# walaj/SeqLib

Measured on AMD Instinct MI355X. Metric: aligned reads/sec (150 bp) via BWAAligner, higher is better.
Workload: dtype int32

## Files before the change

### seqlib_amd/csrc/dev_ext_lane.h

```cpp
#pragma once
#include "dev_seed4.h"
#include "dev_ext_reg.h"
#include "dev_lane_rows.h"

struct alignas(8) LaneJob {
    int64_t s_rbeg, rmax0, rmax1;
    uint64_t q_off;
    int l_query, s_qbeg, s_len, rid;
    float frac_rep;
    int out;
    int r, c;
};

#define LANE_SCORE_LIMIT 16000


struct LaneBases {
    const DevRef &R;
    const uint8_t *query;
    RWin rw;
    __device__ __forceinline__ int q(int j) const { return (int)query[j]; }
    __device__ __forceinline__ int t(int64_t p) { return text_at(R, p, rw); }
};

__device__ __forceinline__ void lane_exits_add(unsigned int *dst, unsigned int mine, int lane)
{
    const unsigned int sum = (unsigned int)__builtin_amdgcn_readlane(dpp_incl_add_scan((int)mine), WAVE - 1);
    if (dst && sum && lane == 0) atomicAdd(dst, sum);
}

template <typename L>
__device__ DReg lane_extend_core(const DevRef &R, const slx_opt &opt, const MatRows &mr, const uint8_t *query, int l_query, int s_qbeg, int s_len,
                                 int64_t s_rbeg, int64_t rmax0, int64_t rmax1, int rid, float frac_rep, L &eh, int row_exit, unsigned int &n_exit)
{
    DReg a;
    a.rb = a.re = 0; a.qb = a.qe = 0; a.sub = a.csub = a.sub_n = 0; a.seedcov = 0; a.secondary = 0;
    a.n_comp = 0; a.hash = 0;
    int aw0 = opt.w, aw1 = opt.w;
    a.w = opt.w; a.rid = rid;
    a.score = a.truesc = s_len * opt.a; a.qb = 0; a.rb = s_rbeg;
    const int qe = s_qbeg + s_len;
    const int64_t re0 = s_rbeg + s_len;
    a.qe = l_query; a.re = re0;
    LaneSide sd[2];
    sd[0].qlen = s_qbeg; sd[0].tlen = (int)(s_rbeg - rmax0); sd[0].q0 = s_qbeg - 1; sd[0].t0 = s_rbeg - 1; sd[0].end_bonus = opt.pen_clip5;
    sd[1].qlen = l_query - qe; sd[1].tlen = (int)(rmax1 - re0); sd[1].q0 = qe; sd[1].t0 = re0; sd[1].end_bonus = opt.pen_clip3;
    LaneBases bases{R, query, {0, -1}};
    lane_rows_extend(sd, s_len * opt.a, opt, mr, eh, bases, [&](int side, const LaneRes &er) {
        if (side == 0) {
            aw0 = er.aw;
            a.score = er.score;
            if (er.gscore <= 0 || er.gscore <= a.score - opt.pen_clip5) { a.qb = s_qbeg - er.qle; a.rb = s_rbeg - er.tle; a.truesc = a.score; }
            else { a.qb = 0; a.rb = s_rbeg - er.gtle; a.truesc = er.gscore; }
        } else {
            aw1 = er.aw;
            const int sc0 = a.score;
            a.score = er.score;
            if (er.gscore <= 0 || er.gscore <= a.score - opt.pen_clip3) { a.qe = qe + er.qle; a.re = re0 + er.tle; a.truesc += a.score - sc0; }
            else { a.qe = l_query; a.re = re0 + er.gtle; a.truesc += er.gscore - sc0; }
        }
    }, row_exit ? EXT_ROW_EXIT_RELAXED : EXT_ROW_EXIT_OFF, &n_exit);
    a.w = aw0 > aw1 ? aw0 : aw1;
    a.seedlen0 = s_len;
    a.frac_rep = frac_rep;
    return a;
}

template <int MAXQ>
__global__ void __launch_bounds__(64) k_cand_lane_prep(DevRef R, Chunk ck, DevOpt dopt, const int *heavy, const unsigned int *n_heavy, const unsigned int *job_off, LaneJob *jobs)
{
    const slx_opt &opt = dopt.o;
    const int lane = threadIdx.x;
    __shared__ int gap_lut[MAXQ + 2];
    for (int q = lane; q < MAXQ + 2; q += WAVE) gap_lut[q] = dev_cal_max_gap(opt, q);
    __syncthreads();
    auto max_gap_of = [&](int q) { return gap_lut[q < 0 ? 0 : (q > MAXQ + 1 ? MAXQ + 1 : q)]; };
    const int64_t l_pac = R.l_pac;
    const unsigned int nh = (unsigned int)__builtin_amdgcn_readfirstlane((int)*n_heavy);
    for (unsigned int s = blockIdx.x; s < nh; s += gridDim.x) {
        const int r = heavy[s];
        const int base = __builtin_amdgcn_readfirstlane(ck.cand_base[r]);
        if (base < 0 || job_off[s + 1] == job_off[s]) continue;
        const unsigned int job0 = job_off[s];
        const ReadWS w = make_ws_uniform(ck, r);
        const uint64_t q_off = ck.offs[r];
        const int l_query = (int)(ck.offs[r + 1] - q_off);
        const int n_chn = ck.n_chain[r];
        const float frac_rep = ck.frac_rep[r];
        unsigned int running = 0;
        for (int cb = 0; cb < n_chn; cb += WAVE) {
            const int ci = cb + lane;
            const int c = ci < n_chn ? w.ia[ci] : -1;
            const int n = c >= 0 ? w.c_n[c] : 0;
            int incl = n;
            for (int d = 1; d < WAVE; d <<= 1) { const int u = __shfl_up(incl, d, WAVE); if (lane >= d) incl += u; }
            const unsigned int my = running + (unsigned int)(incl - n);
            running += (unsigned int)__shfl(incl, WAVE - 1, WAVE);
            if (n <= 0) continue;
            const int *cs = w.c_w + w.c_first[c];
            int64_t rmax0 = l_pac << 1, rmax1 = 0;
            for (int i = 0; i < n; ++i) {
                const int sd = cs[i];
                const int qb = w.s_qbeg(sd), sl = w.s_len(sd);
                const int64_t b = w.s_rbeg[sd] - (qb + max_gap_of(qb));
                const int64_t e = w.s_rbeg[sd] + sl + ((l_query - qb - sl) + max_gap_of(l_query - qb - sl));
                rmax0 = rmax0 < b ? rmax0 : b;
                rmax1 = rmax1 > e ? rmax1 : e;
            }
            rmax0 = rmax0 > 0 ? rmax0 : 0;
            rmax1 = rmax1 < l_pac << 1 ? rmax1 : l_pac << 1;
            const int64_t first_rbeg = w.s_rbeg[cs[0]];
            if (rmax0 < l_pac && l_pac < rmax1) {
                if (first_rbeg < l_pac) rmax1 = l_pac; else rmax0 = l_pac;
            }
            {
                int is_rev;
                const int rid = dev_pos2rid(R, dev_depos(R, first_rbeg, &is_rev));
                int64_t far_beg = R.ann_off[rid], far_end = far_beg + R.ann_len[rid];
                if (is_rev) { const int64_t t = far_beg; far_beg = (l_pac << 1) - far_end; far_end = (l_pac << 1) - t; }
                rmax0 = rmax0 > far_beg ? rmax0 : far_beg;
                rmax1 = rmax1 < far_end ? rmax1 : far_end;
            }
            const int rid_c = w.c_rid[c];
            for (int i = 0; i < n; ++i) {
                const int sd = cs[i];
                LaneJob j;
                j.s_rbeg = w.s_rbeg[sd]; j.rmax0 = rmax0; j.rmax1 = rmax1; j.q_off = q_off; j.l_query = l_query;
                j.s_qbeg = w.s_qbeg(sd); j.s_len = w.s_len(sd); j.rid = rid_c; j.frac_rep = frac_rep; j.out = base + sd; j.r = r; j.c = c;
                jobs[job0 + my + (unsigned int)i] = j;
            }
        }
    }
}

template <typename L>
__global__ void __launch_bounds__(64) k_ext_lanes(DevRef R, Chunk ck, DevOpt dopt, const unsigned int *n_heavy, const unsigned int *job_off, unsigned int *queue,
                                                   const LaneJob *jobs, DReg *cand, int cols)
{
    const slx_opt &opt = dopt.o;
    const int lane = threadIdx.x;
    const MatRows mr = make_matrows(opt.mat);
    extern __shared__ uint32_t lane_lds[];
    L row;
    row.init(lane_lds, cols, lane);
    const unsigned int nh = (unsigned int)__builtin_amdgcn_readfirstlane((int)*n_heavy);
    const unsigned int n_jobs = nh ? (unsigned int)__builtin_amdgcn_readfirstlane((int)job_off[nh]) : 0u;
    unsigned int exit_cnt = 0;
    for (;;) {
        const unsigned int base = wave_take(queue, (unsigned int)WAVE);
        if (base >= n_jobs) break;
        const unsigned int job = base + (unsigned int)lane;
        if (job < n_jobs) {
            const LaneJob j = jobs[job];
            const uint8_t *query = ck.codes + j.q_off;
            DReg a = lane_extend_core<L>(R, opt, mr, query, j.l_query, j.s_qbeg, j.s_len, j.s_rbeg, j.rmax0, j.rmax1, j.rid, j.frac_rep, row, ck.ext_row_exit, exit_cnt);
            const ReadWS w = make_ws(ck, j.r);
            const int n = w.c_n[j.c];
            const int *cs = w.c_w + w.c_first[j.c];
            int cov = 0;
            for (int i = 0; i < n; ++i) {
                const int t = cs[i];
                const int t_qbeg = w.s_qbeg(t), t_len = w.s_len(t);
                const int64_t t_rbeg = w.s_rbeg[t];
                if (t_qbeg >= a.qb && t_qbeg + t_len <= a.qe && t_rbeg >= a.rb && t_rbeg + t_len <= a.re) cov += t_len;
            }
            a.seedcov = cov;
            cand[j.out] = a;
        }
    }
    lane_exits_add(ck.ext_exits, exit_cnt, lane);
}

__device__ __forceinline__ int first_job_bin(const FirstJob &j, int max_len)
{
    const int left = j.s_qbeg, right = j.l_query - j.s_qbeg - j.s_len;
    const float w = sqrtf((float)(left * left + right * right));
    int b = (int)(w * 64.f / (float)(max_len > 0 ? max_len : 1));
    b = b > 63 ? 63 : (b < 0 ? 0 : b);
    return 63 - b;
}
__global__ void __launch_bounds__(256) k_first_bin_count(const FirstJob *jobs, const unsigned int *dp_list, const unsigned int *n_dp, int max_len, unsigned int *bins)
{
    __shared__ unsigned int s[64];
    if (threadIdx.x < 64) s[threadIdx.x] = 0;
    __syncthreads();
    const unsigned int n = *n_dp;
    for (unsigned int t = blockIdx.x * blockDim.x + threadIdx.x; t < n; t += gridDim.x * blockDim.x) atomicAdd(&s[first_job_bin(jobs[dp_list[t]], max_len)], 1u);
    __syncthreads();
    if (threadIdx.x < 64 && s[threadIdx.x]) atomicAdd(&bins[threadIdx.x], s[threadIdx.x]);
}
__global__ void k_first_bin_scan(unsigned int *bins)
{
    if (blockIdx.x == 0 && threadIdx.x == 0) { unsigned int acc = 0; for (int b = 0; b < 64; ++b) { bins[64 + b] = acc; acc += bins[b]; } }
}
__global__ void __launch_bounds__(256) k_first_bin_scatter(const FirstJob *jobs, const unsigned int *dp_list, const unsigned int *n_dp, int max_len, unsigned int *bins, unsigned int *out)
{
    __shared__ unsigned int s_cnt[64], s_base[64];
    const unsigned int n = *n_dp;
    for (unsigned int t0 = blockIdx.x * blockDim.x; t0 < n; t0 += gridDim.x * blockDim.x) {
        if (threadIdx.x < 64) s_cnt[threadIdx.x] = 0;
        __syncthreads();
        const unsigned int t = t0 + threadIdx.x;
        int b = -1;
        unsigned int job = 0, my = 0;
        if (t < n) { job = dp_list[t]; b = first_job_bin(jobs[job], max_len); my = atomicAdd(&s_cnt[b], 1u); }
        __syncthreads();
        if (threadIdx.x < 64 && s_cnt[threadIdx.x]) s_base[threadIdx.x] = atomicAdd(&bins[64 + threadIdx.x], s_cnt[threadIdx.x]);
        __syncthreads();
        if (b >= 0) out[s_base[b] + my] = job;
        __syncthreads();
    }
}

template <typename L>
__global__ void __launch_bounds__(64) k_first_lanes(DevRef R, Chunk ck, DevOpt dopt, unsigned int *queue, const FirstJob *jobs, DReg *first, const unsigned int *list,
                                                     const unsigned int *n_list, int cols, unsigned int *n_ran)
{
    const slx_opt &opt = dopt.o;
    const int lane = threadIdx.x;
    const MatRows mr = make_matrows(opt.mat);
    extern __shared__ uint32_t lane_lds[];
    L row;
    row.init(lane_lds, cols, lane);
    const unsigned int n_jobs = (unsigned int)__builtin_amdgcn_readfirstlane((int)*n_list);
    unsigned int exit_cnt = 0;
    for (;;) {
        const unsigned int base = wave_take(queue, (unsigned int)WAVE);
        if (base >= n_jobs) break;
        const unsigned int t = base + (unsigned int)lane;
        if (t < n_jobs) {
            const unsigned int job = list[t];
            const FirstJob j = jobs[job];
            const DReg a = lane_extend_core<L>(R, opt, mr, ck.codes + j.q_off, j.l_query, j.s_qbeg, j.s_len, j.s_rbeg, j.rmax0, j.rmax1, j.rid, j.frac_rep, row, ck.ext_row_exit, exit_cnt);
            first[job] = a;
        }
        if (lane == 0) atomicAdd(n_ran, n_jobs - base < (unsigned int)WAVE ? n_jobs - base : (unsigned int)WAVE);
    }
    lane_exits_add(ck.ext_exits, exit_cnt, lane);
}

template <typename QF, typename TF>
__device__ __forceinline__ bool lane_diag_extend(int qlen, QF qf, int tlen, TF tf, const slx_opt &o, const MatRows &mr, int amax, int h0, ExtResult &out)
{
    if (tlen < qlen || qlen > 3 * WAVE || qlen < 1) return false;
    if ((long long)h0 + (long long)qlen * amax >= (1 << 22)) return false;
    const int oe_del = o.o_del + o.e_del, oe_ins = o.o_ins + o.e_ins;
    const int oe = oe_del < oe_ins ? oe_del : oe_ins;
    int loss = 0, run = h0, best = h0, best_p = -1;
    for (int p = 0; p < qlen; ++p) {
        const int t = tf(p), q = qf(p);
        const uint32_t rowp = t == 0 ? mr.packed[0] : t == 1 ? mr.packed[1] : t == 2 ? mr.packed[2] : mr.packed[3];
        const int row4 = t == 0 ? mr.q4[0] : t == 1 ? mr.q4[1] : t == 2 ? mr.q4[2] : mr.q4[3];
        const int sc = q < 4 ? __builtin_amdgcn_sbfe((int)rowp, (uint32_t)q << 3, 8u) : row4;
        loss += amax - sc;
        if (loss > oe - 1) return false;
        run += sc;
        if (run > best) { best = run; best_p = p; }
    }
    if (h0 <= loss) return false;
    out.score = best; out.qle = best_p + 1; out.tle = best_p + 1; out.gtle = qlen; out.gscore = run; out.max_off = 0;
    return true;
}

__global__ void __launch_bounds__(256) k_first_diag(DevRef R, Chunk ck, DevOpt dopt, int n, const unsigned int *first_off, unsigned int cap, const FirstJob *jobs, DReg *first,
                                                    unsigned int *dp_list, unsigned int *n_dp)
{
    const slx_opt &opt = dopt.o;
    const MatRows mr = make_matrows(opt.mat);
    int amax = 0;
    for (int i = 0; i < 25; ++i) amax = amax > opt.mat[i] ? amax : opt.mat[i];
    unsigned int n_jobs = first_off[n];
    if (n_jobs > cap) n_jobs = cap;
    const unsigned int job = blockIdx.x * blockDim.x + threadIdx.x;
    if (job >= n_jobs) return;
    const FirstJob j = jobs[job];
    if (j.l_query <= 0) return;
    const uint8_t *codes = ck.codes;
    QWin qw; qw.bits = 0; qw.chunk = 0xffffffffu;
    RWin rw; rw.bits = 0; rw.chunk = -1;
    DReg a;
    a.rb = a.re = 0; a.qb = a.qe = 0; a.sub = a.csub = a.sub_n = 0; a.seedcov = 0; a.secondary = 0;
    a.n_comp = 0; a.hash = 0;
    a.score = a.truesc = -1; a.rid = j.rid;
    const int aw_ext = ((opt.w >> 1) + (opt.w >> 2)) > 0 ? opt.w : opt.w << 1;
    int aw0 = opt.w, aw1 = opt.w;
    bool ok = true;
    const int s_qbeg = j.s_qbeg, s_len = j.s_len, l_query = j.l_query;
    const int64_t s_rbeg = j.s_rbeg;
    if (s_qbeg) {
        aw0 = aw_ext;
        ExtResult er;
        ok = lane_diag_extend(s_qbeg, [&](int p) { return q_at(codes, j.q_off + (uint64_t)(s_qbeg - 1 - p), qw); }, (int)(s_rbeg - j.rmax0),
                              [&](int t) { return text_at(R, s_rbeg - 1 - t, rw); }, opt, mr, amax, s_len * opt.a, er);
        if (ok) {
            a.score = er.score;
            if (er.gscore <= 0 || er.gscore <= a.score - opt.pen_clip5) { a.qb = s_qbeg - er.qle; a.rb = s_rbeg - er.tle; a.truesc = a.score; }
            else { a.qb = 0; a.rb = s_rbeg - er.gtle; a.truesc = er.gscore; }
        }
    } else { a.score = a.truesc = s_len * opt.a; a.qb = 0; a.rb = s_rbeg; }
    if (ok) {
        if (s_qbeg + s_len != l_query) {
            aw1 = aw_ext;
            const int sc0 = a.score, qe = s_qbeg + s_len;
            const int64_t re0 = s_rbeg + s_len;
            ExtResult er;
            ok = lane_diag_extend(l_query - qe, [&](int p) { return q_at(codes, j.q_off + (uint64_t)(qe + p), qw); }, (int)(j.rmax1 - re0),
                                  [&](int t) { return text_at(R, re0 + t, rw); }, opt, mr, amax, sc0, er);
            if (ok) {
                a.score = er.score;
                if (er.gscore <= 0 || er.gscore <= a.score - opt.pen_clip3) { a.qe = qe + er.qle; a.re = re0 + er.tle; a.truesc += a.score - sc0; }
                else { a.qe = l_query; a.re = re0 + er.gtle; a.truesc += er.gscore - sc0; }
            }
        } else { a.qe = l_query; a.re = s_rbeg + s_len; }
    }
    if (ok) {
        a.w = aw0 > aw1 ? aw0 : aw1;
        a.seedlen0 = s_len;
        a.frac_rep = j.frac_rep;
        first[job] = a;
    } else dp_list[wave_fetch_inc(n_dp)] = job;
}
```

### seqlib_amd/csrc/dev_lane_rows.h

```cpp
#pragma once
#include <stdint.h>
#include <stddef.h>
#if defined(__HIPCC__)
#define LROW_FN __host__ __device__ __forceinline__
#define LROW_M __host__ __device__ __forceinline__
#else
#define LROW_FN static inline
#define LROW_M inline
#endif
#ifndef WAVE
#define WAVE 64
#endif

template <typename O>
LROW_FN int ext_tail_bound0(const O &o, int qlen, int h0, int amax)
{
    if (o.o_del < 0 || o.e_del < 0 || o.o_ins < 0 || o.e_ins < 0) return 0x7fffffff;
    const long long b = (long long)h0 + (long long)qlen * (amax > 0 ? amax : 0) - o.o_del - o.e_del;
    return b > 0x3fffffff ? 0x7fffffff : (int)b;
}
LROW_FN bool ext_tail_done(int b, int max, int gscore) { return b <= max && (b > 0 ? b : 0) < gscore; }

#define EXT_ROW_EXIT_OFF 0
#define EXT_ROW_EXIT_STRICT 1
#define EXT_ROW_EXIT_RELAXED 2
template <typename O>
LROW_FN bool ext_row_exit_ok(const O &o, int qlen, int w, int h0)
{
    if (o.o_del < 0 || o.e_del < 0 || o.o_ins < 0 || o.e_ins < 0) return false;
    return w + 1 >= qlen || (long long)h0 - o.o_ins - o.e_ins - (long long)(w + 1) * o.e_ins <= 0;
}
LROW_FN int ext_row_bound(int m, int hb, int apos, int qlen, int beg, int tlen, int i)
{
    const int a = qlen - beg, b = tlen - 1 - i;
    const int k = a < b ? a : b;
    return (m > hb ? m : hb) + apos * (k > 0 ? k : 0);
}
LROW_FN bool ext_row_done(int U, int max, int gscore, int end_bonus) { return (end_bonus >= 0 && U <= max - end_bonus) || ext_tail_done(U, max, gscore); }

struct LaneWide {
    uint32_t *eh;
    static LROW_M size_t bytes(int cols) { return (size_t)cols * WAVE * 4; }
    LROW_M void init(uint32_t *base, int, int lane) { eh = base + lane; }
    LROW_M void put_all(int j, int h, int e, int q) { eh[j * WAVE] = (uint32_t)h | (uint32_t)e << 14 | (uint32_t)q << 28; }
    LROW_M uint32_t get(int j) const { return eh[j * WAVE]; }
    LROW_M int q_of(uint32_t v, int) const { return (int)(v >> 28); }
    static LROW_M int h_of(uint32_t v) { return (int)(v & 0x3fffu); }
    static LROW_M int e_of(uint32_t v) { return (int)((v >> 14) & 0x3fffu); }
    LROW_M void put(int j, int h, int e, uint32_t old) { eh[j * WAVE] = (uint32_t)h | (uint32_t)e << 14 | (old & 0xf0000000u); }
    static LROW_M bool zero(uint32_t v) { return (v & 0x0fffffffu) == 0; }
};
struct LaneNarrow {
    uint16_t *eh;
    uint32_t *qa;
    static LROW_M size_t bytes(int cols) { return (size_t)cols * WAVE * 2 + (size_t)((cols + 7) / 8) * WAVE * 4; }
    LROW_M void init(uint32_t *base, int cols, int lane) { eh = (uint16_t *)base + lane; qa = base + (size_t)cols * WAVE / 2 + lane; }
    LROW_M void put_all(int j, int h, int e, int q)
    {
        eh[j * WAVE] = (uint16_t)(h | e << 8);
        uint32_t w = (j & 7) ? qa[(j >> 3) * WAVE] : 0u;
        w |= (uint32_t)q << ((j & 7) * 4);
        qa[(j >> 3) * WAVE] = w;
    }
    LROW_M uint32_t get(int j) const { return eh[j * WAVE]; }
    LROW_M int q_of(uint32_t, int j) const { return (int)((qa[(j >> 3) * WAVE] >> ((j & 7) * 4)) & 7u); }
    static LROW_M int h_of(uint32_t v) { return (int)(v & 0xffu); }
    static LROW_M int e_of(uint32_t v) { return (int)(v >> 8); }
    LROW_M void put(int j, int h, int e, uint32_t) { eh[j * WAVE] = (uint16_t)(h | e << 8); }
    static LROW_M bool zero(uint32_t v) { return v == 0; }
};

struct LaneSide { int qlen, tlen, q0, end_bonus; int64_t t0; };
struct LaneRes { int score, qle, tle, gtle, gscore, max_off, aw; };

template <typename L, typename F, typename O, typename MR, typename D>
LROW_FN void lane_rows_extend(const LaneSide s[2], int h0, const O &o, const MR &mr, L &row, F &fetch, D done, int row_exit = EXT_ROW_EXIT_STRICT,
                              unsigned int *n_exit = nullptr)
{
    const int o_del = o.o_del, e_del = o.e_del, o_ins = o.o_ins, e_ins = o.e_ins, zdrop = o.zdrop;
    const int oe_del = o_del + e_del, oe_ins = o_ins + e_ins;
    int amax = 0;
    for (int i = 0; i < 25; ++i) amax = amax > o.mat[i] ? amax : o.mat[i];
    int side = s[0].qlen > 0 ? 0 : (s[1].qlen > 0 ? 1 : 2), trial = 0, prev = -1;
    bool fresh = true;
    int qlen = 0, tlen = 0, q0 = 0, dir = 0, w = 0, aw = 0, tail_top = 0, exit_bonus = -1;
    bool exit_ok = false;
    const int apos = amax > 0 ? amax : 0;
    int64_t t0 = 0;
    int max = 0, max_i = -1, max_j = -1, max_ie = -1, gscore = -1, max_off = 0, beg = 0, end = 0, i = 0;
    while (side < 2) {
        if (fresh) {
            fresh = false;
            const int end_bonus = side ? s[1].end_bonus : s[0].end_bonus;
            qlen = side ? s[1].qlen : s[0].qlen; tlen = side ? s[1].tlen : s[0].tlen; q0 = side ? s[1].q0 : s[0].q0; t0 = side ? s[1].t0 : s[0].t0;
            dir = side ? 1 : -1;
            aw = o.w << trial;
            for (int j = 0; j <= qlen; ++j) {
                const int v = h0 - oe_ins - (j - 1) * e_ins;
                const int h = j == 0 ? h0 : (v > 0 ? v : 0);
                row.put_all(j, h, 0, j < qlen ? fetch.q(q0 + dir * j) : 0);
            }
            w = aw;
            int max_ins = (int)((double)(qlen * amax + end_bonus - o_ins) / e_ins + 1.);
            max_ins = max_ins > 1 ? max_ins : 1;
            w = w < max_ins ? w : max_ins;
            int max_del = (int)((double)(qlen * amax + end_bonus - o_del) / e_del + 1.);
            max_del = max_del > 1 ? max_del : 1;
            w = w < max_del ? w : max_del;
            tail_top = ext_tail_bound0(o, qlen, h0, amax);
            exit_ok = row_exit != EXT_ROW_EXIT_OFF && ext_row_exit_ok(o, qlen, w, h0);
            exit_bonus = row_exit == EXT_ROW_EXIT_RELAXED ? end_bonus : -1;
            max = h0;
            max_i = -1; max_j = -1; max_ie = -1; gscore = -1; max_off = 0; beg = 0; end = qlen; i = 0;
        }
        bool stop = i >= tlen || (i >= qlen && ext_tail_done(tail_top - (i - qlen) * e_del, max, gscore));
        if (!stop) {
            const int t = fetch.t(t0 + (int64_t)(dir * i));
            const uint32_t rowp = t == 0 ? mr.packed[0] : t == 1 ? mr.packed[1] : t == 2 ? mr.packed[2] : t == 3 ? mr.packed[3] : mr.packed[4];
            const int row4 = t == 0 ? mr.q4[0] : t == 1 ? mr.q4[1] : t == 2 ? mr.q4[2] : t == 3 ? mr.q4[3] : mr.q4[4];
            int f = 0, m = 0, mj = -1;
            if (beg < i - w) beg = i - w;
            if (end > i + w + 1) end = i + w + 1;
            if (end > qlen) end = qlen;
            int h1 = 0;
            if (beg == 0) { h1 = h0 - (o_del + e_del * (i + 1)); if (h1 < 0) h1 = 0; }
            const int hb = h1;
            uint32_t cur = beg < end ? row.get(beg) : 0u;
            for (int j = beg; j < end; ++j) {
                const uint32_t nxt = row.get(j + 1);
                int M = L::h_of(cur), e = L::e_of(cur);
                const uint32_t q = (uint32_t)row.q_of(cur, j);
#if defined(__HIP_DEVICE_COMPILE__)
                const int sc = q < 4 ? __builtin_amdgcn_sbfe((int)rowp, q << 3, 8u) : row4;
#else
                const int sc = q < 4 ? (int)(int8_t)(rowp >> (q << 3)) : row4;
#endif
                M = M ? M + sc : 0;
                int h = M > e ? M : e;
                h = h > f ? h : f;
                const int hl = h1;
                h1 = h;
                mj = m > h ? mj : j;
                m = m > h ? m : h;
                int t2 = M - oe_del; t2 = t2 > 0 ? t2 : 0;
                e -= e_del; e = e > t2 ? e : t2;
                row.put(j, hl, e, cur);
                t2 = M - oe_ins; t2 = t2 > 0 ? t2 : 0;
                f -= e_ins; f = f > t2 ? f : t2;
                cur = nxt;
            }
            row.put(end, h1, 0, beg < end ? cur : row.get(end));
            if ((end > beg ? end : beg) == qlen) {
                max_ie = gscore > h1 ? max_ie : i;
                gscore = gscore > h1 ? gscore : h1;
            }
            if (m == 0) stop = true;
            else if (m > max) {
                max = m; max_i = i; max_j = mj;
                const int off = mj - i < 0 ? i - mj : mj - i;
                max_off = max_off > off ? max_off : off;
            } else if (zdrop > 0) {
                if (i - max_i > mj - max_j) { if (max - m - ((i - max_i) - (mj - max_j)) * e_del > zdrop) stop = true; }
                else { if (max - m - ((mj - max_j) - (i - max_i)) * e_ins > zdrop) stop = true; }
            }
            if (!stop) {
                int j;
                for (j = beg; j < end && L::zero(row.get(j)); ++j) {}
                beg = j;
                for (j = end; j >= beg && L::zero(row.get(j)); --j) {}
                end = j + 2 < qlen ? j + 2 : qlen;
                if (exit_ok && ext_row_done(ext_row_bound(m, beg == 0 ? hb : 0, apos, qlen, beg, tlen, i), max, gscore, exit_bonus)) {
                    stop = true;
                    if (n_exit) ++*n_exit;
                }
                ++i;
            }
        }
        if (stop) {
            fresh = true;
            const int before = trial ? prev : (side ? h0 : -1);
            if (trial == 0 && !(max == before || max_off < (aw >> 1) + (aw >> 2))) { prev = max; trial = 1; }
            else {
                LaneRes r;
                r.score = max; r.qle = max_j + 1; r.tle = max_i + 1; r.gtle = max_ie + 1; r.gscore = gscore; r.max_off = max_off; r.aw = aw;
                done(side, r);
                if (side == 0) h0 = max;
                side = side == 0 && s[1].qlen > 0 ? 1 : 2;
                trial = 0;
            }
        }
    }
}
```

### seqlib_amd/csrc/slx_align.hip

```cpp
#include <hip/hip_runtime.h>
#include <hipcub/hipcub.hpp>
#include <chrono>
#include <cmath>
#include <functional>
#include <unistd.h>
#include <cstdio>
#include <cstdlib>
#include <cstring>
#include <algorithm>
#include <mutex>
#include <string>
#include <thread>
#include <type_traits>
#include <vector>
#include "slx_internal.h"
#include "dev_seed4.h"
#include "dev_fin.h"
#include "dev_ext_wave.h"
#include "dev_ext_reg.h"
#include "dev_ext_lane.h"
#include "dev_ext_block.h"
#include "dev_ext_seg.h"
#include "dev_fin2.h"
#include "dev_chain_coop.h"
// ... 187 lines not shown
    if (al->rep_k <= 0 || al->rep_k > 31 || !al->have_dense || al->host_idx->seq_len < 1024) return SLX_OK;
    uint64_t bits = 1ull << 20;
    while (bits < al->host_idx->seq_len * 8ull) bits <<= 1;
    while (al->d_rep.ensure(bits / 8) != SLX_OK) {
        (void)hipGetLastError();
        bits >>= 1;
        if (bits < al->host_idx->seq_len || bits < (1ull << 20)) { al->d_rep.release(); return SLX_OK; }
    }
    HIPCHK(hipMemsetAsync(al->d_rep.p, 0, bits / 8, al->stream));
    DevFM<I> fm = fm_of<I>(al);
    fm.sa_dense = al->d_sa_dense.as<I>();
    hipLaunchKernelGGL(k_rep_filter<I>, dim3(al->n_cu * 64), dim3(256), 0, al->stream, fm, al->ref, al->rep_k, al->d_rep.as<uint32_t>(), bits - 1);
    HIPCHK(hipGetLastError());
    HIPCHK(slx_wait_stream(al->stream));
    al->rep_mask = bits - 1;
    return SLX_OK;
}

#define SLX_MAX_WORKERS 8
static int env_hw_queues() { const char *e = getenv("GPU_MAX_HW_QUEUES"); const int v = e ? atoi(e) : 0; return v > 0 ? v : 4; }

static int default_workers()
{
    if (const char *e = getenv("SEQLIB_AMD_WORKERS")) { const int v = atoi(e); if (v >= 1 && v <= SLX_MAX_WORKERS) return v; }
    return 3;
}

static int make_worker_stream(slx_aligner *al, Worker *wk)
{
    if (al->stream_prio) {
        int least = 0, greatest = 0;
        HIPCHK(hipDeviceGetStreamPriorityRange(&least, &greatest));
        HIPCHK(hipStreamCreateWithPriority(&wk->stream, hipStreamNonBlocking, greatest));
    } else HIPCHK(hipStreamCreateWithFlags(&wk->stream, hipStreamNonBlocking));
    return SLX_OK;
}

static int set_seed_stream(slx_aligner *al, Worker *wk)
{
    if (wk->seed_stream) { HIPCHK(slx_wait_stream(wk->seed_stream)); HIPCHK(hipStreamDestroy(wk->seed_stream)); wk->seed_stream = nullptr; }
    if (al->seed_free_cus <= 0) return SLX_OK;
    const int words = (al->n_cu + 31) / 32;
    std::vector<uint32_t> mask((size_t)words, 0u);
    for (int cu = 0; cu < al->n_cu; ++cu)
        if ((cu & 31) < 32 - al->seed_free_cus) mask[(size_t)(cu >> 5)] |= 1u << (cu & 31);
    HIPCHK(hipExtStreamCreateWithCUMask(&wk->seed_stream, (uint32_t)words, mask.data()));
    if (!wk->ev_seed_in) HIPCHK(hipEventCreateWithFlags(&wk->ev_seed_in, hipEventDisableTiming));
    if (!wk->ev_seed_out) HIPCHK(hipEventCreateWithFlags(&wk->ev_seed_out, hipEventDisableTiming));
    return SLX_OK;
}

static int add_worker(slx_aligner *al)
{
    Worker *wk = new Worker();
    wk->id = (int)al->workers.size();
    wk->collect();
    al->workers.push_back(wk);
    { const int rc = make_worker_stream(al, wk); if (rc != SLX_OK) return rc; }
    { const int rc = set_seed_stream(al, wk); if (rc != SLX_OK) return rc; }
    HIPCHK(hipHostMalloc((void **)&wk->h_mail, 256, hipHostMallocDefault));
    for (int b = 0; b < 6; ++b) HIPCHK(hipEventCreate(&wk->dbg_ev[b]));
    for (int i = 0; i <= SLX_N_STAGES; ++i) HIPCHK(hipEventCreate(&wk->ev[i]));
    for (int i = 0; i < 6; ++i) HIPCHK(hipEventCreate(&wk->ev_probe[i]));
    return SLX_OK;
}

static int aligner_init(slx_aligner *al, const slx_index *idx, const int *devices, int n_dev)
{
    al->device = (devices && n_dev > 0) ? devices[0] : 0;
    if (!(devices && n_dev > 0)) (void)hipGetDevice(&al->device);
    HIPCHK(hipSetDevice(al->device));
    hipDeviceProp_t prop;
    HIPCHK(hipGetDeviceProperties(&prop, al->device));
    al->n_cu = prop.multiProcessorCount;
    al->max_threads = al->n_cu * al->threads_per_cu;
    int rcw;
    al->n_workers = default_workers();
    al->hw_queues = env_hw_queues();
    for (int k = 0; k < al->n_workers; ++k) if ((rcw = add_worker(al)) != SLX_OK) return rcw;
    HIPCHK(hipStreamCreateWithFlags(&al->stream, hipStreamNonBlocking));
    al->host_idx = idx;
    int rc;
    if ((rc = al->d_bwt.ensure(idx->bwt.size() * 4 + 64)) != SLX_OK) return rc;
    HIPCHK(hipMemcpy(al->d_bwt.p, idx->bwt.data(), idx->bwt.size() * 4, hipMemcpyHostToDevice));
    if ((rc = al->d_sa_samp.ensure(idx->sa.size() * 8)) != SLX_OK) return rc;
    HIPCHK(hipMemcpy(al->d_sa_samp.p, idx->sa.data(), idx->sa.size() * 8, hipMemcpyHostToDevice));
    al->wide = idx->seq_len + 1 >= (1ULL << 32);
    if ((rc = al->wide ? upload_fm<uint64_t>(al) : upload_fm<uint32_t>(al)) != SLX_OK) return rc;
    if ((rc = al->d_pac.ensure(idx->pac.size() + 16)) != SLX_OK) return rc;
    HIPCHK(hipMemcpy(al->d_pac.p, idx->pac.data(), idx->pac.size(), hipMemcpyHostToDevice));
    std::vector<int64_t> aoff; std::vector<int32_t> alen;
    for (const slx_ann &a : idx->anns) { aoff.push_back(a.offset); alen.push_back(a.len); }
    if ((rc = al->d_ann_off.ensure(aoff.size() * 8 + 8)) != SLX_OK) return rc;
    if ((rc = al->d_ann_len.ensure(alen.size() * 4 + 8)) != SLX_OK) return rc;
    HIPCHK(hipMemcpy(al->d_ann_off.p, aoff.data(), aoff.size() * 8, hipMemcpyHostToDevice));
    HIPCHK(hipMemcpy(al->d_ann_len.p, alen.data(), alen.size() * 4, hipMemcpyHostToDevice));
    al->ref.pac = al->d_pac.as<uint8_t>();
    al->ref.l_pac = idx->l_pac;
    al->ref.n_seqs = (int)idx->anns.size();
    al->ref.ann_off = al->d_ann_off.as<int64_t>();
    al->ref.ann_len = al->d_ann_len.as<int32_t>();
    {
        std::vector<uint8_t> alt;
        bool any = false;
        for (const slx_ann &a : idx->anns) { alt.push_back(a.is_alt ? 1 : 0); any = any || a.is_alt; }
        al->ref.ann_alt = nullptr;
        if (any) {
            if ((rc = al->d_ann_alt.ensure(alt.size() + 8)) != SLX_OK) return rc;
            HIPCHK(hipMemcpy(al->d_ann_alt.p, alt.data(), alt.size(), hipMemcpyHostToDevice));
            al->ref.ann_alt = al->d_ann_alt.as<uint8_t>();
        }
    }
    if ((rc = al->wide ? find_text_is_pac<uint64_t>(al) : find_text_is_pac<uint32_t>(al)) != SLX_OK) return rc;
    if ((rc = al->wide ? build_rep_filter<uint64_t>(al) : build_rep_filter<uint32_t>(al)) != SLX_OK) return rc;
    const int LUT_N = SLX_LOG_LUT_N;
    std::vector<double> lut((size_t)LUT_N);
    lut[0] = -INFINITY;
    for (int i = 1; i < LUT_N; ++i) lut[(size_t)i] = log((double)i);
    if ((rc = al->d_loglut.ensure((size_t)LUT_N * 8)) != SLX_OK) return rc;
    HIPCHK(hipMemcpy(al->d_loglut.p, lut.data(), (size_t)LUT_N * 8, hipMemcpyHostToDevice));
    return SLX_OK;
}


static std::mutex g_live_mu;
static int g_live_aligners = 0;
static void pin_pool_release_all();

static int create_one(const slx_index *idx, int device, bool current, slx_aligner **out)
{
    slx_aligner *al = new slx_aligner();
    { std::lock_guard<std::mutex> g(g_live_mu); ++g_live_aligners; }
    const int rc = aligner_init(al, idx, current ? nullptr : &device, current ? 0 : 1);
    if (rc != SLX_OK) { slx_aligner_free(al); return rc; }
    *out = al;
    return SLX_OK;
}

extern "C" int slx_device_count(void)
{
    int ndev = 0;
    if (hipGetDeviceCount(&ndev) != hipSuccess) { (void)hipGetLastError(); return 0; }
    return ndev;
}

extern "C" int slx_aligner_create(const slx_index *idx, const int *devices, int n_dev, slx_aligner **out)
{
    if (!out) return SLX_EINVAL;
    *out = nullptr;
    if (!idx) { slx_set_error("slx_aligner_create: index is null"); return SLX_EINVAL; }
    const int ndev = slx_device_count();
    if (ndev == 0) {
        slx_set_error("no HIP device: the BWAAligner hot path runs on MI355X only (no CPU fallback)");
        return SLX_ENODEVICE;
    }
    if (n_dev < 0 || (n_dev > 0 && !devices)) { slx_set_error("slx_aligner_create: bad device list"); return SLX_EINVAL; }
    for (int i = 0; i < n_dev; ++i)
        if (devices[i] < 0 || devices[i] >= ndev) { slx_set_error("slx_aligner_create: device %d is not one of the %d visible", devices[i], ndev); return SLX_EINVAL; }
    if (n_dev <= 1) return create_one(idx, n_dev ? devices[0] : 0, n_dev == 0, out);
    slx_aligner *grp = new slx_aligner();
    grp->is_group = true;
    grp->subs.assign((size_t)n_dev, nullptr);
    grp->host_idx = idx;
    std::vector<int> rcs((size_t)n_dev, SLX_OK);
    std::vector<std::string> errs((size_t)n_dev);
    std::vector<std::thread> th;
    for (int i = 0; i < n_dev; ++i)
        th.emplace_back([&, i]() {
            rcs[(size_t)i] = create_one(idx, devices[i], false, &grp->subs[(size_t)i]);
            if (rcs[(size_t)i] != SLX_OK) errs[(size_t)i] = slx_last_error();
        });
    for (auto &t : th) t.join();
    for (int i = 0; i < n_dev; ++i)
        if (rcs[(size_t)i] != SLX_OK) {
            slx_set_error("device %d: %s", devices[i], errs[(size_t)i].c_str());
            const int rc = rcs[(size_t)i];
            slx_aligner_free(grp);
            return rc;
        }
    *out = grp;
    return SLX_OK;
}

extern "C" void slx_aligner_free(slx_aligner *al)
{
    if (!al) return;
    if (al->is_group) {
        for (slx_aligner *sub : al->subs) slx_aligner_free(sub);
        delete al;
        return;
    }
    (void)hipSetDevice(al->device);
    DevBuf *bufs[] = {&al->d_bwt, &al->d_occ, &al->d_sup, &al->d_lut, &al->d_rep, &al->d_sa_samp, &al->d_sa_dense, &al->d_pac, &al->d_ann_off, &al->d_ann_len, &al->d_ann_alt, &al->d_loglut, &al->o_hit_off,
                      &al->o_rid, &al->o_pos, &al->o_flag, &al->o_mapq, &al->o_score, &al->o_nm, &al->o_na, &al->o_ncig, &al->o_cig_off, &al->o_cigar, &al->o_xa, &al->o_sub,
                      &al->st_bases, &al->st_offs, &al->st_pack};
    for (DevBuf *b : bufs) b->release();
    for (Worker *wk : al->workers) {
        for (DevBuf *b : wk->all) b->release();
        for (int i = 0; i <= SLX_N_STAGES; ++i) if (wk->ev[i]) (void)hipEventDestroy(wk->ev[i]);
        for (int i = 0; i < 6; ++i) if (wk->dbg_ev[i]) (void)hipEventDestroy(wk->dbg_ev[i]);
        for (int i = 0; i < 6; ++i) if (wk->ev_probe[i]) (void)hipEventDestroy(wk->ev_probe[i]);
        if (wk->h_mail) (void)hipHostFree(wk->h_mail);
        if (wk->stream) (void)hipStreamDestroy(wk->stream);
        if (wk->seed_stream) (void)hipStreamDestroy(wk->seed_stream);
        if (wk->ev_seed_in) (void)hipEventDestroy(wk->ev_seed_in);
        if (wk->ev_seed_out) (void)hipEventDestroy(wk->ev_seed_out);
        delete wk;
    }
    if (al->h_bounce) (void)hipHostFree(al->h_bounce);
    if (al->stream) (void)hipStreamDestroy(al->stream);
    delete al;
    bool last;
    { std::lock_guard<std::mutex> g(g_live_mu); last = --g_live_aligners == 0; }
    if (last) pin_pool_release_all();
}

extern "C" int slx_aligner_set(slx_aligner *al, const char *key, int64_t value)
{
    if (!al || !key) return SLX_EINVAL;
    if (al->is_group) {
        std::lock_guard<std::mutex> call(al->call_mu);
        for (slx_aligner *sub : al->subs) { const int rc = slx_aligner_set(sub, key, value); if (rc != SLX_OK) return rc; }
        return SLX_OK;
    }
    std::lock_guard<std::mutex> call(al->call_mu);
    if (!strcmp(key, "chunk_reads")) { if (value < 1) return SLX_EINVAL; al->chunk_reads = value; }
    else if (!strcmp(key, "cap_intv")) { if (value < 1) return SLX_EINVAL; al->cap_intv = (int)value; }
    else if (!strcmp(key, "dense_sa")) al->dense_sa = value != 0;
    else if (!strcmp(key, "wide_index")) {
        const bool want = value != 0 || al->host_idx->seq_len + 1 >= (1ULL << 32);
        if (want != al->wide) {
            HIPCHK(hipSetDevice(al->device));
            al->wide = want;
            int rc = want ? upload_fm<uint64_t>(al) : upload_fm<uint32_t>(al);
            if (rc != SLX_OK) return rc;
            if ((rc = want ? build_rep_filter<uint64_t>(al) : build_rep_filter<uint32_t>(al)) != SLX_OK) return rc;
        }
    }
    else if (!strcmp(key, "chain_mode")) al->chain_mode = (int)value;
    else if (!strcmp(key, "keep_stages")) al->keep_stages = (int)value;
    else if (!strcmp(key, "lut_k")) {
        if (value != 0 && value != -1 && (value < 2 || value > 14)) return SLX_EINVAL;
        al->lut_k = (int)value;
        (void)hipSetDevice(al->device);
        return al->wide ? build_lut<uint64_t>(al) : build_lut<uint32_t>(al);
    }
    else if (!strcmp(key, "cand_mode")) al->cand_mode = (int)value;
    else if (!strcmp(key, "cand_seeds")) { if (value < 1) return SLX_EINVAL; al->cand_seeds = (int)value; }
    else if (!strcmp(key, "heavy_sorted")) al->heavy_sorted = (int)value;
    else if (!strcmp(key, "ext_split")) al->ext_split = (int)value;
    else if (!strcmp(key, "coop_lim1")) { if (value < 1) return SLX_EINVAL; al->coop_lim1 = (int)value; }
    else if (!strcmp(key, "coop_lim2")) { if (value < 1) return SLX_EINVAL; al->coop_lim2 = (int)value; }
    else if (!strcmp(key, "long_coop")) al->long_coop = value != 0;
    else if (!strcmp(key, "long_seed3")) al->long_seed3 = value != 0;
    else if (!strcmp(key, "long_predict")) al->long_predict = value != 0;
    else if (!strcmp(key, "long_block")) { if (value < 0 || value > (1 << 24)) return SLX_EINVAL; al->long_block = (int)value; }
    else if (!strcmp(key, "long_guess")) al->long_guess = value != 0;
    else if (!strcmp(key, "long_seg")) al->long_seg = value != 0;
    else if (!strcmp(key, "bwd_direct")) al->bwd_direct = value != 0;
    else if (!strcmp(key, "xseg_wave_min")) { if (value < 0) return SLX_EINVAL; al->xseg_wave_min = (int)value; }
    else if (!strcmp(key, "xseg_fail")) { if (value < 0) return SLX_EINVAL; al->xseg_fail = (int)value; }
    else if (!strcmp(key, "long_budget")) { if (value < 0 || value > (1 << 20)) return SLX_EINVAL; al->long_budget = (int)value; }
    else if (!strcmp(key, "regs_big")) { if (value < 2) return SLX_EINVAL; al->regs_big = (int)value; }
    else if (!strcmp(key, "regs_defer")) al->regs_defer = value != 0;
    else if (!strcmp(key, "hits_wave")) al->hits_wave = value != 0;
    else if (!strcmp(key, "cig_fast_coop")) al->cig_fast_coop = value != 0;
    else if (!strcmp(key, "cig_lane_il")) al->cig_lane_il = value != 0;
    else if (!strcmp(key, "small_coop")) al->small_coop = value != 0;
    else if (!strcmp(key, "small_spread")) al->small_spread = value != 0;
    else if (!strcmp(key, "chain_sorted")) al->chain_sorted = value != 0;
    else if (!strcmp(key, "regs_sorted")) al->regs_sorted = value != 0;
    else if (!strcmp(key, "cand_top")) { if (value < 0) return SLX_EINVAL; al->cand_top = (int)value; }
    else if (!strcmp(key, "cand_rep_max")) { if (value < 0) return SLX_EINVAL; al->cand_rep_max = (int)value; }
    else if (!strcmp(key, "cand_rep")) { if (value < -1 || value > 101) return SLX_EINVAL; al->cand_rep = (int)value; }
    else if (!strcmp(key, "cand_lanes")) { if (value < -1 || value > 1) return SLX_EINVAL; al->cand_lanes = (int)value; }
    else if (!strcmp(key, "cig_lanes")) al->cig_lanes = value != 0;
    else if (!strcmp(key, "first_diag")) al->first_diag = value != 0;
    else if (!strcmp(key, "first_lanes")) al->first_lanes = value != 0;
    else if (!strcmp(key, "chain_lds")) al->chain_lds = value != 0;
    else if (!strcmp(key, "lane_narrow")) al->lane_narrow = value != 0;
    else if (!strcmp(key, "lane_pad")) al->lane_pad = (int)value;
    else if (!strcmp(key, "cand_lane_seeds")) { if (value < 1) return SLX_EINVAL; al->cand_lane_seeds = (int)value; }
    else if (!strcmp(key, "cand_cap")) { if (value < 1) return SLX_EINVAL; al->cand_cap = (int)value; }
    else if (!strcmp(key, "split_min")) al->split_min = (int)value;
    else if (!strcmp(key, "heavy_seeds")) { if (value < 1) return SLX_EINVAL; al->heavy_seeds = (int)value; }
    else if (!strcmp(key, "workers")) {
        if (value < 1 || value > SLX_MAX_WORKERS) return SLX_EINVAL;
        HIPCHK(hipSetDevice(al->device));
        while ((int)al->workers.size() < (int)value) { const int rc = add_worker(al); if (rc != SLX_OK) return rc; }
        al->n_workers = (int)value;
    }
    else if (!strcmp(key, "min_split")) { if (value < 1) return SLX_EINVAL; al->min_split = value; }
    else if (!strcmp(key, "seed_quota")) { if (value < 0 || value > (1 << 24)) return SLX_EINVAL; al->seed_quota = (int)value; }
    else if (!strcmp(key, "rep_k")) {
        if (value < 0 || value > 31) return SLX_EINVAL;
        al->rep_k = (int)value;
        HIPCHK(hipSetDevice(al->device));
        return al->wide ? build_rep_filter<uint64_t>(al) : build_rep_filter<uint32_t>(al);
    }
    else if (!strcmp(key, "top_heavy")) al->top_heavy = value != 0;
    else if (!strcmp(key, "top_reuse")) al->top_reuse = value != 0;
    else if (!strcmp(key, "walk_stage")) al->walk_stage = value != 0;
    else if (!strcmp(key, "ext_row_exit")) al->ext_row_exit = value != 0;
    else if (!strcmp(key, "p2_items")) al->p2_items = value != 0;
    else if (!strcmp(key, "p2_coop")) al->p2_coop = value != 0;
    else if (!strcmp(key, "p2_items_cap")) al->p2_items_cap = (int)value;
    else if (!strcmp(key, "seed_free_cus")) {
        if (value < 0 || value > 24) return SLX_EINVAL;
        HIPCHK(hipSetDevice(al->device));
        al->seed_free_cus = (int)value;
        for (Worker *wk : al->workers) { const int rc = set_seed_stream(al, wk); if (rc != SLX_OK) return rc; }
    }
    else if (!strcmp(key, "stream_prio")) {
        if (value < 0 || value > 1) return SLX_EINVAL;
        HIPCHK(hipSetDevice(al->device));
        al->stream_prio = (int)value;
        for (Worker *wk : al->workers) {
            HIPCHK(slx_wait_stream(wk->stream));
            HIPCHK(hipStreamDestroy(wk->stream));
            wk->stream = nullptr;
            const int rc = make_worker_stream(al, wk);
            if (rc != SLX_OK) return rc;
        }
    }
    else if (!strcmp(key, "threads")) { if (value < 64) return SLX_EINVAL; al->max_threads = (int)value; }
    else if (!strcmp(key, "zarena_bytes")) { if (value < 1024) return SLX_EINVAL; al->zcap = (unsigned long long)value; }
    else if (!strcmp(key, "z_start") || !strcmp(key, "cig_start")) {
        if (value < 0 || value > (1ll << 32)) return SLX_EINVAL;
        (key[0] == 'z' ? al->z_start : al->cig_start) = (unsigned long long)value;
        al->z_hook = al->cig_hook = 0;
    }
    else { slx_set_error("slx_aligner_set: unknown key %s", key); return SLX_EINVAL; }
    return SLX_OK;
}

extern "C" int slx_aligner_stage_ms(const slx_aligner *al, float ms[SLX_N_STAGES])
{
    if (!al || !ms) return SLX_EINVAL;
    if (al->is_group) {
        for (int i = 0; i < SLX_N_STAGES; ++i) { ms[i] = 0; for (const slx_aligner *sub : al->subs) ms[i] = std::max(ms[i], sub->stage_ms[i]); }
        return SLX_OK;
    }
    for (int i = 0; i < SLX_N_STAGES; ++i) ms[i] = al->stage_ms[i];
    return SLX_OK;
}

extern "C" int slx_aligner_probe_ms(const slx_aligner *al, float ms[SLX_N_PROBES], int64_t *n_reads)
{
    if (!al || !ms) return SLX_EINVAL;
    if (al->is_group) {
        int64_t n = 0;
        for (int i = 0; i < SLX_N_PROBES; ++i) ms[i] = 0;
        for (const slx_aligner *sub : al->subs) { for (int i = 0; i < SLX_N_PROBES; ++i) ms[i] += sub->probe_ms[i]; n += sub->probe_reads; }
        if (n_reads) *n_reads = n;
        return SLX_OK;
    }
    for (int i = 0; i < SLX_N_PROBES; ++i) ms[i] = al->probe_ms[i];
    if (n_reads) *n_reads = al->probe_reads;
    return SLX_OK;
}

extern "C" int64_t slx_aligner_counter(const slx_aligner *al, const char *key)
{
    if (!al || !key) return -1;
    if (!strcmp(key, "workers")) return al->is_group ? al->subs[0]->n_workers : al->n_workers;
    if (!strcmp(key, "text_is_pac")) return (al->is_group ? al->subs[0] : al)->text_is_pac ? 1 : 0;
    if (!strcmp(key, "hw_queues")) return al->hw_queues;
    if (!strcmp(key, "long_rounds") || !strcmp(key, "long_jobs")) {
        long long v = 0;
        const bool rounds = key[5] == 'r';
        auto take = [&](const slx_aligner *a) { for (const Worker *wk : a->workers) v = std::max(v, rounds ? (long long)wk->long_rounds_run : (long long)wk->long_jobs_run); };
        if (al->is_group) for (const slx_aligner *sub : al->subs) take(sub); else take(al);
        return v;
    }
    {
        if (!strcmp(key, "pseg_jobs")) {
            long long v = 0;
            auto take = [&](const slx_aligner *a) { for (const Worker *wk : a->workers) v += wk->pseg_stat; };
            if (al->is_group) for (const slx_aligner *sub : al->subs) take(sub); else take(al);
            return v;
        }
        if (!strcmp(key, "chain_lds_bail") || !strcmp(key, "chain_lds_reads")) {
            long long v = 0;
            const int which = key[10] == 'r';
            auto take = [&](const slx_aligner *a) { for (const Worker *wk : a->workers) v += (long long)wk->chain_stat[which]; };
            if (al->is_group) for (const slx_aligner *sub : al->subs) take(sub); else take(al);
            return v;
        }
        if (!strcmp(key, "first_lane_jobs")) {
            long long v = 0;
            auto take = [&](const slx_aligner *a) { for (const Worker *wk : a->workers) v += (long long)wk->first_stat; };
            if (al->is_group) for (const slx_aligner *sub : al->subs) take(sub); else take(al);
            return v;
        }
        if (!strcmp(key, "walk_staged_chains")) {
            long long v = 0;
            auto take = [&](const slx_aligner *a) { for (const Worker *wk : a->workers) v += (long long)wk->walk_stat; };
            if (al->is_group) for (const slx_aligner *sub : al->subs) take(sub); else take(al);
            return v;
        }
        if (!strcmp(key, "ext_row_exits")) {
            long long v = 0;
            auto take = [&](const slx_aligner *a) { for (const Worker *wk : a->workers) v += (long long)wk->exit_stat; };
            if (al->is_group) for (const slx_aligner *sub : al->subs) take(sub); else take(al);
            return v;
        }
        if (!strcmp(key, "retries")) {
            long long v = 0;
            if (al->is_group) for (const slx_aligner *sub : al->subs) v += sub->n_retries; else v = al->n_retries;
            return v;
        }
        if (!strcmp(key, "ovf_sites")) {
            long long v = 0;
            if (al->is_group) for (const slx_aligner *sub : al->subs) v |= (long long)sub->ovf_sites; else v = (long long)al->ovf_sites;
            return v;
        }
        if (!strcmp(key, "guard_dirty")) {
            long long v = 0;
            if (al->is_group) for (const slx_aligner *sub : al->subs) v += sub->guard_dirty; else v = al->guard_dirty;
            return v;
        }
        if (!strcmp(key, "regs_deferred") || !strcmp(key, "hits_wave_reads")) {
            long long v = 0;
            const int which = key[0] == 'h';
            auto take = [&](const slx_aligner *a) { for (const Worker *wk : a->workers) v += (long long)wk->fin_stat[which]; };
            if (al->is_group) for (const slx_aligner *sub : al->subs) take(sub); else take(al);
            return v;
        }
        static const char *const gs[3] = {"gseg_ok", "gseg_redo", "gseg_jobs"};
        for (int i = 0; i < 3; ++i)
            if (!strcmp(key, gs[i])) {
                long long v = 0;
                auto take = [&](const slx_aligner *a) { for (const Worker *wk : a->workers) v += wk->gseg_stat[i]; };
                if (al->is_group) for (const slx_aligner *sub : al->subs) take(sub); else take(al);
                return v;
            }
        static const char *const xs[4] = {"xseg_ok", "xseg_redo", "xseg_retry", "xseg_sides"};
        for (int i = 0; i < 4; ++i)
            if (!strcmp(key, xs[i])) {
                long long v = 0;
                auto take = [&](const slx_aligner *a) { for (const Worker *wk : a->workers) v += wk->xseg_stat[i]; };
                if (al->is_group) for (const slx_aligner *sub : al->subs) take(sub); else take(al);
                return v;
            }
    }
    if (!strcmp(key, "group_merge_us")) return al->merge_us;
    if (!strcmp(key, "group_call_us")) return al->call_us;
    static const char *const names[4] = {"heavy_reads", "p2_calls", "p2_coop_calls", "p2_whole_reads"};
    for (int i = 0; i < 4; ++i)
        if (!strcmp(key, names[i])) {
            if (!al->is_group) return al->counters[i];
            long long n = 0;
            for (const slx_aligner *sub : al->subs) n += sub->counters[i];
            return n;
        }
    return -1;
}

extern "C" int slx_aligner_probe_launches(const slx_aligner *al)
{
    if (!al) return 0;
    if (al->is_group) { int n = 0; for (const slx_aligner *sub : al->subs) n += sub->probe_launches; return n; }
    return al->probe_launches;
}

#include "slx_chunk.inc"


__global__ void k_shift_offsets(int64_t *dst, const int64_t *src, int64_t n, int64_t add)
{
    int64_t i = (int64_t)blockIdx.x * blockDim.x + threadIdx.x;
    if (i < n) dst[i] = src[i] + add;
}

#define SLX_GUARD_BYTES (1u << 20)
#define SLX_GUARD_FILL 0xa5
__global__ void k_guard_count(const uint8_t *z_tail, const uint8_t *cig_tail, unsigned long long *dirty)
{
    const size_t at = ((size_t)blockIdx.x * blockDim.x + threadIdx.x) * 8;
    if (at >= SLX_GUARD_BYTES) return;
    unsigned int d = 0;
    for (int k = 0; k < 8; ++k) d += (z_tail[at + k] != SLX_GUARD_FILL) + (cig_tail[at + k] != SLX_GUARD_FILL);
    if (d) atomicAdd(dirty, (unsigned long long)d);
}

static int guard_arm(Worker *wk, const ChunkCaps &caps)
{
    int rc;
    if ((rc = wk->zarena.ensure((size_t)caps.zcap + SLX_GUARD_BYTES)) != SLX_OK) return rc;
    if ((rc = wk->cigpool.ensure((size_t)caps.cigcap * 4 + SLX_GUARD_BYTES)) != SLX_OK) return rc;
    if ((rc = wk->guard_cnt.ensure(8)) != SLX_OK) return rc;
    HIPCHK(hipMemsetAsync(wk->zarena.as<uint8_t>() + caps.zcap, SLX_GUARD_FILL, SLX_GUARD_BYTES, wk->stream));
    HIPCHK(hipMemsetAsync(wk->cigpool.as<uint8_t>() + caps.cigcap * 4, SLX_GUARD_FILL, SLX_GUARD_BYTES, wk->stream));
    return SLX_OK;
}

static int attempt_report(Worker *wk, const ChunkCaps &caps, bool hook, uint32_t *quiet, unsigned long long *dirty)
{
    *quiet = 0; *dirty = 0;
    if (hook) {
        HIPCHK(hipMemsetAsync(wk->guard_cnt.p, 0, 8, wk->stream));
        hipLaunchKernelGGL(k_guard_count, dim3(SLX_GUARD_BYTES / 8 / 256), dim3(256), 0, wk->stream, (const uint8_t *)wk->zarena.as<uint8_t>() + caps.zcap,
                           (const uint8_t *)wk->cigpool.as<uint8_t>() + caps.cigcap * 4, wk->guard_cnt.as<unsigned long long>());
        HIPCHK(hipMemcpyAsync(dirty, wk->guard_cnt.p, 8, hipMemcpyDeviceToHost, wk->stream));
    }
    HIPCHK(hipMemcpyAsync(quiet, wk->counters.as<uint32_t>() + 5, 4, hipMemcpyDeviceToHost, wk->stream));
    HIPCHK(slx_wait_stream(wk->stream));
    return SLX_OK;
}

template <typename I>
static int worker_run(slx_aligner *al, Worker *wk, const slx_opt *opt, const uint8_t *d_bases, const uint64_t *d_offs, int64_t r_lo, int64_t r_hi,
                      uint64_t rng_state, uint64_t first_ordinal, int hardclip, double keepSecFrac, int maxSecondary, const char *h_bases, const uint64_t *h_offs)
{
    HIPCHK(hipSetDevice(al->device));
    if (h_offs && r_hi > r_lo) {
        const uint64_t b0 = h_offs[r_lo], b1 = h_offs[r_hi];
        if (b0 < al->h_first || b1 < b0 || b1 > al->h_last) { slx_set_error("read offsets are not monotonic (part [%lld, %lld))", (long long)r_lo, (long long)r_hi); return SLX_EINVAL; }
        if (b1 > b0) HIPCHK(hipMemcpyAsync((void *)(d_bases + b0), h_bases + b0, b1 - b0, hipMemcpyHostToDevice, wk->stream));
        HIPCHK(hipMemcpyAsync((void *)(d_offs + r_lo), h_offs + r_lo, ((size_t)(r_hi - r_lo) + 1) * 8, hipMemcpyHostToDevice, wk->stream));
    }
    for (int i = 0; i < SLX_N_STAGES; ++i) wk->stage_ms[i] = 0;
    for (int i = 0; i < SLX_N_PROBES; ++i) wk->probe_ms[i] = 0;
    wk->n_chunks = 0;
    for (long long &c : wk->cnt) c = 0;
    wk->chain_stat[0] = wk->chain_stat[1] = 0;
    wk->first_stat = 0;
    wk->walk_stat = 0;
    wk->exit_stat = 0;
    int rc;
    const int64_t n_part = r_hi - r_lo;
    if ((rc = wk->o_hit_off.ensure(((size_t)n_part + 1) * 8)) != SLX_OK) return rc;
    if ((rc = wk->len_stat.ensure(32)) != SLX_OK) return rc;
    int64_t hit_base = 0, cig_base = 0;
    for (int64_t r0 = r_lo, step = 0; r0 < r_hi; r0 += step) {
        const int n = (int)std::min<int64_t>(al->chunk_reads, r_hi - r0);
        step = n;
        unsigned long long stat[4] = {0, 0, 0, 0};
        HIPCHK(hipMemsetAsync(wk->len_stat.p, 0, 32, wk->stream));
        hipLaunchKernelGGL(k_len_stats, dim3((unsigned)((n + 255) / 256)), dim3(256), 0, wk->stream, d_offs + r0, n, wk->len_stat.as<unsigned long long>());
        { MailSpec ms{}; ms.src[0] = wk->len_stat.as<unsigned int>(); ms.words[0] = 8; ms.n = 1;
          hipLaunchKernelGGL(k_mail, dim3(1), dim3(64), 0, wk->stream, ms, wk->h_mail); }
        HIPCHK(slx_wait_stream(wk->stream));
        memcpy(stat, wk->h_mail, 32);
        if (stat[1]) { slx_set_error("read offsets are not monotonic in reads [%lld, %lld)", (long long)r0, (long long)(r0 + n)); return SLX_EINVAL; }
        const int max_len = (int)std::min<unsigned long long>(stat[0], 1u << 30);
        if (max_len > SLX_MAX_READ_LEN) {
            slx_set_error("read of %d bp: the GPU path supports reads up to %d bp", max_len, SLX_MAX_READ_LEN);
            return SLX_EUNSUPPORTED;
        }
        uint64_t pair[2] = {stat[2], stat[3]};
        ChunkCaps caps;
        bool hook = false;
        {
            std::lock_guard<std::mutex> g(al->mu);
            caps.cap_intv = al->cap_intv;
            caps.zcap = std::max<unsigned long long>(al->zcap, (unsigned long long)n * al->z_per_read);
            if (max_len > 704) {
                caps.cap_intv = std::max(std::max(caps.cap_intv, al->cap_intv_long), max_len / 8 + 64);
                caps.zcap = std::max(caps.zcap, std::min<unsigned long long>((unsigned long long)n * (unsigned long long)max_len * 208ull, 4ull << 30));
            }
            caps.cigcap = std::max<unsigned long long>(al->cig_floor, (unsigned long long)n * al->cig_per_read + 4096);
            hook = al->z_start != 0 || al->cig_start != 0;
        }
        const unsigned long long lane_blocks = (unsigned long long)std::min<long long>((long long)al->n_cu * 16, (long long)n * 4 / 64 + 1);
        const unsigned long long z_waves = (unsigned long long)std::min(n, al->n_cu * 32) * CIG_WAVE_Z +
                                           (al->cig_lane_il ? lane_blocks * ((unsigned long long)LANE_IL_WORDS(max_len) * 256ull + 255ull) : 0ull);
        const unsigned long long cig_waves = (unsigned long long)std::min(n, al->n_cu * 32) * CIG_WAVE_WORDS;
        caps.zcap += z_waves; caps.cigcap += cig_waves;
        if (hook) {
            std::lock_guard<std::mutex> g(al->mu);
            if (al->z_start) caps.zcap = al->z_start;
            if (al->cig_start) caps.cigcap = al->cig_start;
            caps.zcap = std::max(caps.zcap, al->z_hook); caps.cigcap = std::max(caps.cigcap, al->cig_hook);
        }
        for (int attempt = 0;; ++attempt) {
            uint32_t fl = 0;
            int64_t hb = hit_base, cb = cig_base;
            if (hook && (rc = guard_arm(wk, caps)) != SLX_OK) return rc;
            if (max_len > SLX_NARROW_MAX_LEN)
                rc = sizeof(I) == 8 ? slx_run_chunk_wide_u64(al, wk, opt, d_bases, d_offs, pair, r0, r_lo, n, max_len, rng_state, first_ordinal, hardclip, keepSecFrac, maxSecondary,
                                                             caps, &hb, &cb, &fl)
                                    : slx_run_chunk_wide_u32(al, wk, opt, d_bases, d_offs, pair, r0, r_lo, n, max_len, rng_state, first_ordinal, hardclip, keepSecFrac, maxSecondary,
                                                             caps, &hb, &cb, &fl);
            else
            rc = run_chunk<I>(al, wk, opt, d_bases, d_offs, pair, r0, r_lo, n, max_len, rng_state, first_ordinal, hardclip, keepSecFrac, maxSecondary,
                              caps, &hb, &cb, &fl);
            if (rc != SLX_OK) return rc;
            if (hook || fl) {
                uint32_t quiet = 0;
                unsigned long long dirty = 0;
                if ((rc = attempt_report(wk, caps, hook, &quiet, &dirty)) != SLX_OK) return rc;
                std::lock_guard<std::mutex> g(al->mu);
                al->ovf_sites |= (fl & OVS_MASK) | quiet;
                al->guard_dirty += (long long)dirty;
            }
            if (!fl) {
                hit_base = hb; cig_base = cb;
                ++wk->n_chunks;
                std::lock_guard<std::mutex> g(al->mu);
                if (max_len > 704) al->cap_intv_long = std::max(al->cap_intv_long, caps.cap_intv);
                else al->cap_intv = std::max(al->cap_intv, caps.cap_intv);
                if (attempt > 0) {
                    if (hook) { al->z_hook = std::max(al->z_hook, caps.zcap); al->cig_hook = std::max(al->cig_hook, caps.cigcap); }
                    else if (n >= 65536) {
                        al->z_per_read = std::max<unsigned long long>(al->z_per_read, (caps.zcap - z_waves + n - 1) / (unsigned long long)n);
                        al->cig_per_read = std::max<unsigned long long>(al->cig_per_read, (caps.cigcap - cig_waves + n - 1) / (unsigned long long)n);
                    } else {
                        al->zcap = std::max(al->zcap, caps.zcap - z_waves);
                        al->cig_floor = std::max(al->cig_floor, caps.cigcap - cig_waves);
                    }
                }
                al->n_retries += attempt;
                break;
            }
            if (getenv("SLX_DEBUG_RETRY")) fprintf(stderr, "[retry] worker %d reads %lld+%d attempt %d flags 0x%x (cap_intv %d zcap %llu cigcap %llu)\n", wk->id,
                                                   (long long)r0, n, attempt, fl, caps.cap_intv, caps.zcap, caps.cigcap);
            if (fl & (ERR_LOGLUT | ERR_INTERNAL)) { slx_set_error("device pipeline error flags 0x%x", fl); return SLX_EINTERNAL; }
            if (attempt >= 12) { slx_set_error("chunk still overflows its work areas after %d retries (flags 0x%x)", attempt, fl); return SLX_ENOMEM; }
            if (fl & OVF_INTV) caps.cap_intv *= 2;
            if (fl & OVF_ZARENA) caps.zcap *= 2;
            if (fl & OVF_CIGAR) caps.cigcap *= 2;
        }
    }
    {
        int64_t last[1] = {hit_base};
        HIPCHK(hipMemcpyAsync(wk->o_hit_off.as<int64_t>() + n_part, last, 8, hipMemcpyHostToDevice, wk->stream));
        if ((rc = wk->o_cig_off.grow(((size_t)hit_base + 2) * 8, (size_t)hit_base * 8, wk->stream)) != SLX_OK) return rc;
        int64_t lastc[1] = {cig_base};
        HIPCHK(hipMemcpyAsync(wk->o_cig_off.as<int64_t>() + hit_base, lastc, 8, hipMemcpyHostToDevice, wk->stream));
        HIPCHK(slx_wait_stream(wk->stream));
    }
    wk->n_hits = hit_base; wk->n_cig = cig_base;
    return SLX_OK;
}

struct EventPair {
    hipEvent_t t0 = nullptr, t1 = nullptr;
    ~EventPair() { if (t0) (void)hipEventDestroy(t0); if (t1) (void)hipEventDestroy(t1); }
};

static int align_device_locked(slx_aligner *al, const slx_opt *opt, const void *d_bases, const void *d_offs_, int64_t n_reads,
                               uint64_t rng_state, uint64_t first_ordinal, int hardclip, double keepSecFrac, int maxSecondary, slx_hits *out,
                               const char *h_bases = nullptr, const uint64_t *h_offs = nullptr)
{
    memset(out, 0, sizeof *out);
    HIPCHK(hipSetDevice(al->device));
    if (opt->e_del <= 0 || opt->e_ins <= 0) { slx_set_error("gap extension penalty must be > 0 on the GPU path (bwa divides by it)"); return SLX_EINVAL; }
    const uint64_t *d_offs = (const uint64_t *)d_offs_;
    const int K = (n_reads >= 2 * al->min_split) ? std::min<int>(al->n_workers, (int)al->workers.size()) : 1;
    al->active_k = K;
    EventPair tp;
    HIPCHK(hipEventCreate(&tp.t0)); HIPCHK(hipEventCreate(&tp.t1));
    HIPCHK(hipEventRecord(tp.t0, al->stream));
    HIPCHK(slx_wait_stream(al->stream));
    std::vector<int64_t> lo((size_t)K + 1);
    for (int k = 0; k <= K; ++k) lo[(size_t)k] = n_reads * k / K;
    const bool wide = al->wide;
    const bool sam = (opt->flag & SLX_F_REG2SAM) != 0;
    auto run_worker = [=](Worker *wk, int64_t a, int64_t b) {
        return wide ? worker_run<uint64_t>(al, wk, opt, (const uint8_t *)d_bases, d_offs, a, b, rng_state, first_ordinal, hardclip, keepSecFrac, maxSecondary, h_bases, h_offs)
                    : worker_run<uint32_t>(al, wk, opt, (const uint8_t *)d_bases, d_offs, a, b, rng_state, first_ordinal, hardclip, keepSecFrac, maxSecondary, h_bases, h_offs);
    };
    if (K == 1) {
        Worker *wk = al->workers[0];
        wk->rc = run_worker(wk, 0, n_reads);
        if (wk->rc != SLX_OK) return wk->rc;
    } else {
        std::vector<std::thread> th;
        for (int k = 0; k < K; ++k) {
            Worker *wk = al->workers[(size_t)k];
            const int64_t a = lo[(size_t)k], b = lo[(size_t)k + 1];
            th.emplace_back([=]() {
                wk->rc = run_worker(wk, a, b);
                if (wk->rc != SLX_OK) wk->err = slx_last_error();
            });
        }
        for (auto &t : th) t.join();
        for (int k = 0; k < K; ++k)
            if (al->workers[(size_t)k]->rc != SLX_OK) { slx_set_error("%s", al->workers[(size_t)k]->err.c_str()); return al->workers[(size_t)k]->rc; }
    }
    for (int i = 0; i < SLX_N_STAGES; ++i) {
        al->stage_ms[i] = 0;
        for (int k = 0; k < K; ++k) al->stage_ms[i] += al->workers[(size_t)k]->stage_ms[i];
    }
    al->probe_reads = n_reads;
    al->probe_launches = 0;
    for (int k = 0; k < K; ++k) al->probe_launches += al->workers[(size_t)k]->n_chunks;
    for (int i = 0; i < 4; ++i) { al->counters[i] = 0; for (int k = 0; k < K; ++k) al->counters[i] += al->workers[(size_t)k]->cnt[i]; }
    for (int i = 0; i < SLX_N_PROBES; ++i) {
        al->probe_ms[i] = 0;
        for (int k = 0; k < K; ++k) al->probe_ms[i] += al->workers[(size_t)k]->probe_ms[i];
    }
    slx_hits r;
    memset(&r, 0, sizeof r);
    r.n_reads = n_reads; r.on_device = 1;
    if (K == 1) {
        Worker *wk = al->workers[0];
        r.n_hits = wk->n_hits; r.n_cigar = wk->n_cig;
        r.hit_off = wk->o_hit_off.as<int64_t>(); r.rid = wk->o_rid.as<int32_t>(); r.pos = wk->o_pos.as<int64_t>();
        r.flag = wk->o_flag.as<uint16_t>(); r.mapq = wk->o_mapq.as<uint8_t>(); r.score = wk->o_score.as<int32_t>();
        r.nm = wk->o_nm.as<int32_t>(); r.na = wk->o_na.as<int32_t>(); r.n_cigar_ops = wk->o_ncig.as<int32_t>();
        r.cig_off = wk->o_cig_off.as<int64_t>(); r.cigar = wk->o_cigar.as<uint32_t>();
        if (sam) { r.xa_parent = wk->o_xa.as<int32_t>(); r.sub = wk->o_sub.as<int32_t>(); }
    } else {
        int64_t H = 0, C = 0;
        for (int k = 0; k < K; ++k) { H += al->workers[(size_t)k]->n_hits; C += al->workers[(size_t)k]->n_cig; }
        int rc;
#define ENSO(buf, bytes) if ((rc = al->buf.ensure((size_t)(bytes))) != SLX_OK) return rc
        ENSO(o_hit_off, ((size_t)n_reads + 1) * 8); ENSO(o_rid, ((size_t)H + 1) * 4); ENSO(o_pos, ((size_t)H + 1) * 8); ENSO(o_flag, ((size_t)H + 1) * 2);
        ENSO(o_mapq, (size_t)H + 1); ENSO(o_score, ((size_t)H + 1) * 4); ENSO(o_nm, ((size_t)H + 1) * 4); ENSO(o_na, ((size_t)H + 1) * 4);
        ENSO(o_ncig, ((size_t)H + 1) * 4); ENSO(o_cig_off, ((size_t)H + 2) * 8); ENSO(o_cigar, ((size_t)C + 1) * 4);
        if (sam) { ENSO(o_xa, ((size_t)H + 1) * 4); ENSO(o_sub, ((size_t)H + 1) * 4); }
#undef ENSO
        int64_t hb = 0, cb = 0;
        hipStream_t st = al->stream;
        for (int k = 0; k < K; ++k) {
            Worker *wk = al->workers[(size_t)k];
            const int64_t np = lo[(size_t)k + 1] - lo[(size_t)k], h = wk->n_hits, c = wk->n_cig;
            const int last = k == K - 1 ? 1 : 0;
            hipLaunchKernelGGL(k_shift_offsets, dim3((unsigned)((np + last + 255) / 256)), dim3(256), 0, st, al->o_hit_off.as<int64_t>() + lo[(size_t)k],
                               wk->o_hit_off.as<int64_t>(), np + last, hb);
            hipLaunchKernelGGL(k_shift_offsets, dim3((unsigned)((h + last + 255) / 256)), dim3(256), 0, st, al->o_cig_off.as<int64_t>() + hb,
                               wk->o_cig_off.as<int64_t>(), h + last, cb);
#define CAT(buf, type, cnt, base) if ((cnt) > 0) HIPCHK(hipMemcpyAsync(al->buf.as<type>() + (base), wk->buf.as<type>(), (size_t)(cnt) * sizeof(type), hipMemcpyDeviceToDevice, st))
            CAT(o_rid, int32_t, h, hb); CAT(o_pos, int64_t, h, hb); CAT(o_flag, uint16_t, h, hb); CAT(o_mapq, uint8_t, h, hb); CAT(o_score, int32_t, h, hb);
            CAT(o_nm, int32_t, h, hb); CAT(o_na, int32_t, h, hb); CAT(o_ncig, int32_t, h, hb); CAT(o_cigar, uint32_t, c, cb);
            if (sam) { CAT(o_xa, int32_t, h, hb); CAT(o_sub, int32_t, h, hb); }
#undef CAT
            hb += h; cb += c;
        }
        HIPCHK(hipGetLastError());
        r.n_hits = H; r.n_cigar = C;
        r.hit_off = al->o_hit_off.as<int64_t>(); r.rid = al->o_rid.as<int32_t>(); r.pos = al->o_pos.as<int64_t>();
        r.flag = al->o_flag.as<uint16_t>(); r.mapq = al->o_mapq.as<uint8_t>(); r.score = al->o_score.as<int32_t>();
        r.nm = al->o_nm.as<int32_t>(); r.na = al->o_na.as<int32_t>(); r.n_cigar_ops = al->o_ncig.as<int32_t>();
        r.cig_off = al->o_cig_off.as<int64_t>(); r.cigar = al->o_cigar.as<uint32_t>();
        if (sam) { r.xa_parent = al->o_xa.as<int32_t>(); r.sub = al->o_sub.as<int32_t>(); }
    }
    HIPCHK(hipEventRecord(tp.t1, al->stream));
    HIPCHK(slx_wait_stream(al->stream));
    float tot = 0;
    (void)hipEventElapsedTime(&tot, tp.t0, tp.t1);
    al->stage_ms[7] = tot;
    *out = r;
    return SLX_OK;
}

extern "C" int slx_align_batch_device(slx_aligner *al, const slx_opt *opt, const void *d_bases, const void *d_offs, int64_t n_reads,
                                      uint64_t rng_state, uint64_t first_ordinal, int hardclip, double keepSecFrac, int maxSecondary,
                                      slx_hits *out)
{
    if (!al || !opt || !out || n_reads < 0) { slx_set_error("slx_align_batch_device: bad argument"); return SLX_EINVAL; }
    if (al->is_group) { slx_set_error("slx_align_batch_device: reads resident on one GPU cannot be sharded -- use one aligner per device, or slx_align_batch"); return SLX_EINVAL; }
    std::lock_guard<std::mutex> call(al->call_mu);
    return align_device_locked(al, opt, d_bases, d_offs, n_reads, rng_state, first_ordinal, hardclip, keepSecFrac, maxSecondary, out);
}

namespace {
struct PinBlock { void *p; uint64_t cap; };
std::mutex g_pin_mu;
std::vector<PinBlock> g_pin_pool;
const size_t PIN_KEEP = 4;
const uint64_t PIN_KEEP_BYTES = 8ull << 30;
void *pin_acquire(uint64_t bytes, uint64_t *cap)
{
    {
        std::lock_guard<std::mutex> g(g_pin_mu);
        size_t best = g_pin_pool.size();
        for (size_t i = 0; i < g_pin_pool.size(); ++i)
            if (g_pin_pool[i].cap >= bytes && (best == g_pin_pool.size() || g_pin_pool[i].cap < g_pin_pool[best].cap)) best = i;
        if (best < g_pin_pool.size()) { void *p = g_pin_pool[best].p; *cap = g_pin_pool[best].cap; g_pin_pool.erase(g_pin_pool.begin() + (long)best); return p; }
    }
    void *p = nullptr;
    const uint64_t want = bytes + bytes / 16;
    if (hipHostMalloc(&p, want, hipHostMallocPortable | hipHostMallocMapped) != hipSuccess) { (void)hipGetLastError(); return nullptr; }
    *cap = want;
    return p;
}
void pin_release(void *p, uint64_t cap)
{
    {
        std::lock_guard<std::mutex> g(g_pin_mu);
        uint64_t held = cap;
        for (const PinBlock &b : g_pin_pool) held += b.cap;
        bool alive;
        { std::lock_guard<std::mutex> g2(g_live_mu); alive = g_live_aligners > 0; }
        if (alive && g_pin_pool.size() < PIN_KEEP && held <= PIN_KEEP_BYTES) { g_pin_pool.push_back({p, cap}); return; }
    }
    (void)hipHostFree(p);
}
}
static void pin_pool_release_all()
{
    std::vector<PinBlock> drop;
    { std::lock_guard<std::mutex> g(g_pin_mu); drop.swap(g_pin_pool); }
    for (const PinBlock &b : drop) (void)hipHostFree(b.p);
}

extern "C" void *slx_host_alloc(uint64_t bytes)
{
    void *p = nullptr;
    if (hipHostMalloc(&p, bytes ? bytes : 1, hipHostMallocDefault) != hipSuccess) { (void)hipGetLastError(); slx_set_error("cannot pin %llu bytes of host memory", (unsigned long long)bytes); return nullptr; }
    return p;
}
extern "C" void slx_host_free(void *p) { if (p) (void)hipHostFree(p); }
extern "C" void slx_host_trim(void) { pin_pool_release_all(); }

static uint64_t packed_base(uint64_t N, uint64_t H, uint64_t Cg) { return 32 + 8 * (N + 1) + 8 * H + 8 * (H + 1) + 5 * 4 * H + 4 * Cg + 2 * H + H; }
static uint64_t packed_size(uint64_t N, uint64_t H, uint64_t Cg, bool sam = false) { const uint64_t b = packed_base(N, H, Cg); return sam ? ((b + 3) & ~3ull) + 8 * H : b; }

static int pack_locked(slx_aligner *al, const slx_hits *h, void *dst);

static void view_packed(slx_hits *out, uint8_t *blk, int64_t N, int64_t H, int64_t C, bool sam = false)
{
    uint8_t *d = blk + 32;
    out->hit_off = (int64_t *)d; d += 8 * ((size_t)N + 1);
    out->pos = (int64_t *)d; d += 8 * (size_t)H;
    out->cig_off = (int64_t *)d; d += 8 * ((size_t)H + 1);
    out->rid = (int32_t *)d; d += 4 * (size_t)H;
    out->score = (int32_t *)d; d += 4 * (size_t)H;
    out->nm = (int32_t *)d; d += 4 * (size_t)H;
    out->na = (int32_t *)d; d += 4 * (size_t)H;
    out->n_cigar_ops = (int32_t *)d; d += 4 * (size_t)H;
    out->cigar = (uint32_t *)d; d += 4 * (size_t)C;
    out->flag = (uint16_t *)d; d += 2 * (size_t)H;
    out->mapq = (uint8_t *)d;
    out->xa_parent = out->sub = nullptr;
    if (sam) {
        uint8_t *e = blk + ((packed_base((uint64_t)N, (uint64_t)H, (uint64_t)C) + 3) & ~3ull);
        out->xa_parent = (int32_t *)e; out->sub = (int32_t *)(e + 4 * (size_t)H);
    }
// ... 293 lines not shown
```

### seqlib_amd/csrc/slx_align_types.h

```cpp
#pragma once
#include <hip/hip_runtime.h>
#include <mutex>
#include <string>
#include <vector>
#include "slx_internal.h"
#include "dev_fm.h"
#include "dev_types.h"

#define HIPCHK(x)                                                                                   \
    do {                                                                                            \
        hipError_t e_ = (x);                                                                        \
        if (e_ != hipSuccess) {                                                                     \
            slx_set_error("HIP error %s at %s:%d (%s)", hipGetErrorString(e_), __FILE__, __LINE__, #x); \
            return e_ == hipErrorOutOfMemory ? SLX_ENOMEM : SLX_ENODEVICE;                          \
        }                                                                                           \
    } while (0)

struct DevBuf {
    void *p = nullptr;
    size_t cap = 0;
    int ensure(size_t bytes)
    {
        if (bytes <= cap) return SLX_OK;
        if (p) (void)hipFree(p);
        p = nullptr; cap = 0;
        size_t want = bytes + bytes / 8 + 256;
        HIPCHK(hipMalloc(&p, want));
        cap = want;
        return SLX_OK;
    }
    int grow(size_t bytes, size_t keep, hipStream_t st)
    {
        if (bytes <= cap) return SLX_OK;
        void *q = nullptr;
        size_t want = bytes + bytes / 2 + 256;
        HIPCHK(hipMalloc(&q, want));
        if (p && keep) {
            hipError_t e = hipMemcpyAsync(q, p, keep, hipMemcpyDeviceToDevice, st);
            if (e == hipSuccess) e = hipStreamSynchronize(st);
            if (e != hipSuccess) { (void)hipFree(q); HIPCHK(e); }
        }
        if (p) (void)hipFree(p);
        p = q; cap = want;
        return SLX_OK;
    }
    void release() { if (p) (void)hipFree(p); p = nullptr; cap = 0; }
    template <typename T> T *as() const { return (T *)p; }
};

#define SLX_MAIL_PARTS 8
struct MailSpec { const unsigned int *src[SLX_MAIL_PARTS]; int words[SLX_MAIL_PARTS]; int n; };
static __global__ void k_mail(MailSpec s, unsigned int *dst)
{
    int at = 0;
    for (int i = 0; i < s.n; ++i) {
        for (int w = (int)threadIdx.x; w < s.words[i]; w += (int)blockDim.x) dst[at + w] = s.src[i][w];
        at += s.words[i];
    }
}
struct slx_aligner;
#define SMALL_SPREAD_MAX 512

struct Worker {
    hipStream_t stream = nullptr;
    hipStream_t seed_stream = nullptr;
    hipEvent_t ev_seed_in = nullptr, ev_seed_out = nullptr;
    unsigned int *h_mail = nullptr;
    DevBuf codes, offs_rel, intv_n, intv_info, intv_x0, intv_x2, l_rep, seed_cnt, seed_off, scan_tmp;
    DevBuf s_rbeg, s_ql, s_next, c_pos, c_head, c_tail, c_n, c_rid, c_w, c_first, c_kept, ia, ib, ic, srt, regs, hits;
    DevBuf n_chain, n_reg, n_hit, na, frac_rep, zarena, cigpool, counters, lists, hit_cnt, cig_cnt, hit_off_c, cig_off_c;
    DevBuf order_key_in, order_key_out, order_in, order_out, queues, sort_tmp, jobs, fast_list, dp_list, part_flag, part_pos, cand, cand_base,
        cand_cnt, cand_off, dbg_cyc, order_tmp, first_tab, first_cnt, first_off, fb_list, first_jobs, len_stat, s_score, long_list, long_scratch, huge_rows;
    DevBuf guard_cnt;
    DevBuf chain_left;
    DevBuf order_bin, bin_cnt;
    DevBuf defer_list, hits_big;
    DevBuf first_sorted, first_bins;
    DevBuf p2mask, p2list, p2items, p2long, lane_jobs, first_dp, cig_lane_list;
    DevBuf job_key_in, job_key_out, job_val_in, job_val_out, job_sort_tmp;
    DevBuf seed3_buf;
    DevBuf memo_idx, memo_jobs, memo_tab, round_list, todo_a, todo_b, spec_cnt;
    int long_rounds_run = 0; unsigned int long_jobs_run = 0;
    DevBuf xseg_jobs, xseg_state, xseg_units, xseg_out, xseg_wrec, xseg_wout, xseg_scratch, xseg_cnt;
    DevBuf gseg_jobs, gseg_units, gseg_wrec, gseg_wout, gseg_scratch, gseg_cnt;
    DevBuf pseg_jobs, pseg_idx, pseg_cnt;
    unsigned long long fin_stat[2] = {0, 0};
    unsigned long long chain_stat[2] = {0, 0};
    unsigned long long first_stat = 0;
    bool first_lanes_ran = false;
    unsigned long long walk_stat = 0;
    unsigned long long exit_stat = 0;
    unsigned int pseg_stat = 0;
    unsigned int gseg_stat[3] = {0, 0, 0};
    unsigned int xseg_stat[4] = {0, 0, 0, 0};
    DevBuf snap_ia, snap_regs, snap_nreg;
    Chunk last_ck;
    size_t last_S1 = 0;
    bool last_valid = false, last_wide = false;
    int id = 0;
    unsigned int max_seed_cnt = 0;
    hipEvent_t dbg_ev[6] = {nullptr, nullptr, nullptr, nullptr, nullptr, nullptr};
    DevBuf o_hit_off, o_rid, o_pos, o_flag, o_mapq, o_score, o_nm, o_na, o_ncig, o_cig_off, o_cigar, o_xa, o_sub;
    hipEvent_t ev[SLX_N_STAGES + 1];
    hipEvent_t ev_probe[6] = {nullptr, nullptr, nullptr, nullptr, nullptr, nullptr};
    float stage_ms[SLX_N_STAGES];
    float probe_ms[SLX_N_PROBES] = {0, 0, 0, 0, 0, 0};
    int n_chunks = 0;
    long long cnt[4] = {0, 0, 0, 0};
    int64_t n_hits = 0, n_cig = 0;
    int rc = SLX_OK;
    std::string err;
    std::vector<DevBuf *> all;
    void collect()
    {
        all = {&codes, &offs_rel, &intv_n, &intv_info, &intv_x0, &intv_x2, &l_rep, &seed_cnt, &seed_off, &scan_tmp, &s_rbeg, &s_ql, &s_next,
               &c_pos, &c_head, &c_tail, &c_n, &c_rid, &c_w, &c_first, &c_kept, &ia, &ib, &ic, &srt, &regs, &hits, &n_chain, &n_reg, &n_hit,
               &na, &frac_rep, &zarena, &cigpool, &counters, &lists, &hit_cnt, &cig_cnt, &hit_off_c, &cig_off_c, &order_key_in,
               &order_key_out, &order_in, &order_out, &queues, &sort_tmp, &jobs, &fast_list, &dp_list, &part_flag, &part_pos, &cand, &cand_base,
               &cand_cnt, &cand_off, &dbg_cyc, &order_tmp, &first_tab, &first_cnt, &first_off, &fb_list, &first_jobs, &len_stat, &s_score, &long_list, &long_scratch, &huge_rows, &p2mask, &p2list, &p2items, &p2long, &lane_jobs, &first_dp, &first_sorted, &first_bins, &cig_lane_list, &defer_list, &hits_big, &order_bin, &bin_cnt, &chain_left, &guard_cnt, &snap_ia, &snap_regs, &snap_nreg,
               &memo_idx, &memo_jobs, &memo_tab, &round_list, &todo_a, &todo_b, &spec_cnt, &seed3_buf, &job_key_in, &job_key_out, &job_val_in, &job_val_out, &job_sort_tmp, &pseg_jobs, &pseg_idx, &pseg_cnt, &gseg_jobs, &gseg_units, &gseg_wrec, &gseg_wout, &gseg_scratch, &gseg_cnt, &xseg_jobs, &xseg_state, &xseg_units, &xseg_out, &xseg_wrec, &xseg_wout, &xseg_scratch, &xseg_cnt,
               &o_hit_off, &o_rid, &o_pos, &o_flag, &o_mapq, &o_score, &o_nm, &o_na, &o_ncig, &o_cig_off, &o_cigar, &o_xa, &o_sub};
        for (auto &e : ev) e = nullptr;
    }
};

struct slx_aligner {
    std::vector<slx_aligner *> subs;
    bool is_group = false;
    int64_t merge_us = 0, call_us = 0;
    int device = 0;
    hipStream_t stream = nullptr;
    DevBuf d_bwt, d_occ, d_sup, d_lut, d_rep, d_sa_samp, d_sa_dense, d_pac, d_ann_off, d_ann_len, d_ann_alt, d_loglut;
    uint64_t rep_mask = 0;
    int rep_k = 19;
    bool wide = false;
    DevFM<uint32_t> fm32;
    DevFM<uint64_t> fm64;
    DevRef ref;
    bool dense_sa = true;
    bool have_dense = false;
    bool text_is_pac = true;
    const slx_index *host_idx = nullptr;
    int64_t chunk_reads = 1 << 24;
    int cap_intv = 40;
    int cap_intv_long = 0;
    int long_predict = 0;
    int long_block = 32768;
    int long_seed3 = 1;
    int long_coop = 1;
    int bwd_direct = 0;
    int long_seg = 1;
    int xseg_wave_min = 2048;
    int xseg_fail = 0;
    int long_guess = 0;
    int long_budget = 1024;
    int regs_sorted = 0;
    int chain_sorted = 0;
    int small_spread = 1;
    int cig_fast_coop = 1;
    int cig_lane_il = 1;
    int hits_wave = 1;
    int small_coop = 1;
    int regs_defer = 1;
    int regs_big = 48;
    int coop_lim1 = 1 << 30, coop_lim2 = 1 << 30;
    int ext_split = 1;
    int heavy_sorted = 1;
    int cand_lanes = -1;
    int cand_lane_seeds = 64;
    int cig_lanes = 1;
    int first_lanes = 1;
    int chain_lds = 1;
    int first_diag = 1;
    int lane_narrow = 1;
    int lane_pad = 0;
    int cand_mode = 1;
    int cand_seeds = 256;
    int cand_top = 512;
    int cand_rep = -1;
    int cand_rep_max = 4096;
    int cand_cap = 1 << 23;
    int lut_k = -1;
    int keep_stages = 0;
    int chain_mode = 1;
    int heavy_seeds = 64;
    int split_min = 4096;
    int seed_quota = 0;
    int top_heavy = 0;
    int p2_items = 1;
    int p2_coop = 1;
    int p2_items_cap = 0;
    int top_reuse = 1;
    int walk_stage = 1;
    int ext_row_exit = 1;
    int seed_free_cus = 0;
    int stream_prio = 0;
    int n_workers = 3;
    int hw_queues = 4;
    int active_k = 1;
    int64_t min_split = 1 << 18;
    int max_threads = 0;
    int threads_per_cu = 1536;
    int n_cu = 256;
    unsigned long long zcap = 1ull << 26;
    unsigned long long z_per_read = 512;
    unsigned long long cig_per_read = 8;
    unsigned long long cig_floor = 0;
    int n_retries = 0;
    unsigned long long z_start = 0, cig_start = 0;
    unsigned long long z_hook = 0, cig_hook = 0;
    long long guard_dirty = 0;
    uint32_t ovf_sites = 0;
    std::mutex mu;
    std::mutex call_mu;
    std::vector<Worker *> workers;
    DevBuf o_hit_off, o_rid, o_pos, o_flag, o_mapq, o_score, o_nm, o_na, o_ncig, o_cig_off, o_cigar, o_xa, o_sub;
    DevBuf st_bases, st_offs, st_pack;
    unsigned char *h_bounce = nullptr;
    float stage_ms[SLX_N_STAGES];
    float probe_ms[SLX_N_PROBES] = {0, 0, 0, 0, 0, 0};
    int64_t probe_reads = 0;
    long long counters[4] = {0, 0, 0, 0};
    int probe_launches = 0;
    uint64_t h_first = 0, h_last = 0;
};

template <typename I> static DevFM<I> &fm_of(slx_aligner *al);
template <> DevFM<uint32_t> &fm_of<uint32_t>(slx_aligner *al) { return al->fm32; }
template <> DevFM<uint64_t> &fm_of<uint64_t>(slx_aligner *al) { return al->fm64; }

struct ChunkCaps { int cap_intv; unsigned long long zcap, cigcap; };

#define SLX_LOG_LUT_N (1 << 21)
#define SLX_NARROW_MAX_LEN 65000

int slx_run_chunk_wide_u32(slx_aligner *al, Worker *wk, const slx_opt *opt, const uint8_t *d_ascii, const uint64_t *d_offs, const uint64_t *h_offs_pair,
                           int64_t r0, int64_t part_lo, int n, int max_len, uint64_t rng_state, uint64_t first_ordinal, int hardclip, double ksf, int maxsec,
                           const ChunkCaps &caps, int64_t *hit_base, int64_t *cig_base, uint32_t *flags_out);
int slx_run_chunk_wide_u64(slx_aligner *al, Worker *wk, const slx_opt *opt, const uint8_t *d_ascii, const uint64_t *d_offs, const uint64_t *h_offs_pair,
                           int64_t r0, int64_t part_lo, int n, int max_len, uint64_t rng_state, uint64_t first_ordinal, int hardclip, double ksf, int maxsec,
                           const ChunkCaps &caps, int64_t *hit_base, int64_t *cig_base, uint32_t *flags_out);
```

### seqlib_amd/csrc/slx_chunk.inc

```

__device__ __forceinline__ uint32_t nt4_of(uint32_t b)
{
    const uint32_t u = b & 0xDFu;
    const uint32_t x = (b >> 1) & 3u;
    const bool letter = u == 'A' || u == 'C' || u == 'G' || u == 'T';
    return b < 4u ? b : (letter ? (x ^ (x >> 1)) : 4u);
}

__global__ void k_encode(const uint8_t *ascii, uint8_t *codes, size_t n)
{
    const size_t n16 = (n + 15) >> 4;
    const size_t stride = (size_t)gridDim.x * blockDim.x;
    const bool aligned = ((uintptr_t)ascii & 3) == 0;
    for (size_t t = (size_t)blockIdx.x * blockDim.x + threadIdx.x; t < n16; t += stride) {
        const size_t i = t << 4;
        uint32_t w[4];
        if (aligned && i + 16 <= n) {
            const uint32_t *src = (const uint32_t *)(ascii + i);
#pragma unroll
            for (int k = 0; k < 4; ++k) w[k] = src[k];
        } else {
#pragma unroll
            for (int k = 0; k < 4; ++k) {
                w[k] = 0;
// ... 559 lines not shown
    ck.codes = wk->codes.as<uint8_t>();
    ck.offs = wk->offs_rel.as<uint64_t>();
    ck.first_ordinal = first_ordinal + (uint64_t)r0;
    ck.rng_state = rng_state;
    ck.cap_intv = caps.cap_intv;
    ck.intv_n = wk->intv_n.as<uint32_t>(); ck.intv_info = wk->intv_info.as<uint32_t>();
    ck.intv_x0 = wk->intv_x0.p; ck.intv_x2 = wk->intv_x2.p;
    ck.l_rep = wk->l_rep.as<int32_t>();
    ck.seed_off = wk->seed_off.as<uint64_t>();
    ck.n_chain = wk->n_chain.as<int32_t>(); ck.n_reg = wk->n_reg.as<int32_t>(); ck.n_hit = wk->n_hit.as<int32_t>();
    ck.na = wk->na.as<int32_t>(); ck.frac_rep = wk->frac_rep.as<float>();
    ck.zarena = wk->zarena.as<uint8_t>(); ck.zcap = caps.zcap; ck.zused = wk->counters.as<unsigned long long>();
    ck.cigpool = wk->cigpool.as<uint32_t>(); ck.cigcap = caps.cigcap; ck.cigused = wk->counters.as<unsigned long long>() + 1;
    ck.flags = (uint32_t *)(wk->counters.as<unsigned long long>() + 2);
    ck.log_lut = al->d_loglut.as<double>(); ck.log_lut_n = SLX_LOG_LUT_N;
    ck.lists = wk->lists.p; ck.cap_list = cap_list; ck.n_threads = n_threads;
    ck.hardclip = hardclip; ck.keepSecFrac = ksf; ck.maxSecondary = maxsec;
    ck.sam_mode = (opt->flag & SLX_F_REG2SAM) ? 1 : 0;
    ck.seed_cnt = wk->seed_cnt.as<unsigned long long>();
    ck.ext_row_exit = al->ext_row_exit; ck.ext_exits = wk->queues.as<unsigned int>() + 56;
    const bool production = al->chain_mode == 1 && n >= al->split_min && !has_long;
    const bool use_cand = al->cand_mode == 1 && production;
    if (use_cand) {
        ENS(cand, (size_t)al->cand_cap * sizeof(DReg)); ENS(cand_base, (size_t)n * 4); ENS(cand_cnt, ((size_t)n + 2) * 8); ENS(cand_off, ((size_t)n + 2) * 8);
        HIPCHK(hipMemsetAsync(wk->cand_base.p, 0xff, (size_t)n * 4, st));
        ck.cand = wk->cand.as<DReg>(); ck.cand_base = wk->cand_base.as<int32_t>();
    }
    if (getenv("SLX_DEBUG_CYC")) {
        ENS(dbg_cyc, (size_t)n * 32);
        HIPCHK(hipMemsetAsync(wk->dbg_cyc.p, 0, (size_t)n * 32, st));
        ck.dbg_cyc = wk->dbg_cyc.as<unsigned long long>();
        ck.dbg_stage = atoi(getenv("SLX_DEBUG_CYC"));
    }
    DevOpt dopt; dopt.o = *opt;
    DevFM<I> fm = fm_of<I>(al);
    fm.sa_dense = (al->dense_sa && al->have_dense && al->text_is_pac) ? al->d_sa_dense.as<I>() : nullptr;
    fm.rep = al->rep_mask ? al->d_rep.as<uint32_t>() : nullptr; fm.rep_mask = al->rep_mask; fm.rep_k = al->rep_k;
    fm.bwd_direct = (al->bwd_direct && fm.sa_dense && (sizeof(I) == 8 || (uint64_t)fm.seq_len < (1ULL << 31))) ? 1 : 0;

    (void)hipEventRecord(wk->ev[0], st);
    {
        const unsigned g = (unsigned)std::min<uint64_t>((n_bases / 16 + 255) / 256 + 1, 65535u * 4);
        hipLaunchKernelGGL(k_encode, dim3(g), dim3(256), 0, st, d_ascii + base0, wk->codes.as<uint8_t>(), (size_t)n_bases);
        hipLaunchKernelGGL(k_rel_offsets, dim3((unsigned)((n + 1 + 255) / 256)), dim3(256), 0, st, d_offs + r0, wk->offs_rel.as<uint64_t>(), n, base0);
    }
    (void)hipEventRecord(wk->ev[1], st);
    (void)hipEventRecord(wk->ev_probe[0], st);
    {
        hipStream_t ss = st;
        if (wk->seed_stream && production_seed(al, n, has_long)) {
            ss = wk->seed_stream;
            HIPCHK(hipEventRecord(wk->ev_seed_in, st));
            HIPCHK(hipStreamWaitEvent(ss, wk->ev_seed_in, 0));
        }
        unsigned int *qq = wk->queues.as<unsigned int>();
        hipLaunchKernelGGL((k_seed12m<I, 1>), dim3(seed_grid), dim3(bs), 0, ss, fm, al->ref, ck, dopt, qq + 29, seed_quota,
                           (const int *)nullptr, (const unsigned int *)nullptr, (const unsigned long long *)nullptr, (const uint32_t *)nullptr, (const unsigned int *)nullptr, 0u,
                           (uint32_t *)nullptr, (unsigned int *)nullptr, 0u);
        const uint32_t cap_items = (al->p2_items && n < (1 << 26)) ? (uint32_t)(al->p2_items_cap > 0 ? std::min(al->p2_items_cap, n) : n) : 0u;
        const uint32_t cap_long = (cap_items && al->p2_coop) ? cap_items : 0u;
        hipLaunchKernelGGL(k_seed2_select<I>, dim3((unsigned)(((int64_t)n * spread + bs - 1) / bs)), dim3(bs), 0, ss, fm, ck, dopt, wk->p2mask.as<unsigned long long>(), wk->p2list.as<int>(), qq + 35,
                           wk->p2items.as<uint32_t>(), qq + 37, cap_items);
        hipLaunchKernelGGL((k_seed12m<I, 2>), dim3(grid), dim3(bs), 0, ss, fm, al->ref, ck, dopt, qq + 36, 0u, wk->p2list.as<int>(), qq + 35,
                           wk->p2mask.as<unsigned long long>(), wk->p2items.as<uint32_t>(), qq + 37, cap_items, wk->p2long.as<uint32_t>(), qq + 38, cap_long);
        if (cap_long) hipLaunchKernelGGL(k_seed2_coop<I>, dim3((unsigned)(al->n_cu * 8)), dim3(64), 0, ss, fm, al->ref, ck, dopt, qq + 39, wk->p2long.as<uint32_t>(), qq + 38, cap_long);
        const int seed3_par = (max_len > 8192 && al->long_seed3) ? 4096 : 0x7fffffff;
        hipLaunchKernelGGL(k_seed3m<I>, dim3((unsigned)(((int64_t)n * spread + bs - 1) / bs)), dim3(bs), 0, ss, fm, al->ref, ck, dopt, seed3_par);
        if (seed3_par != 0x7fffffff) {
            ENS(seed3_buf, (size_t)n_bases * sizeof(Seed3Next<I>));
            hipLaunchKernelGGL(k_seed3_next<I>, dim3((unsigned)((n_bases + 255) / 256)), dim3(256), 0, ss, fm, al->ref, ck, dopt, seed3_par, (uint64_t)n_bases, wk->seed3_buf.as<Seed3Next<I>>());
            hipLaunchKernelGGL(k_seed3_chase<I>, dim3((unsigned)((n + 63) / 64)), dim3(64), 0, ss, ck, dopt, seed3_par, (const Seed3Next<I> *)wk->seed3_buf.as<Seed3Next<I>>());
        }
        hipLaunchKernelGGL(k_seed_epi<I>, dim3((unsigned)((n + 63) / 64)), dim3(64), 0, ss, ck, dopt, wk->queues.as<unsigned int>() + 31,
                           (unsigned int)al->heavy_seeds, wk->queues.as<unsigned int>() + 34);
        if (ss != st) {
            HIPCHK(hipEventRecord(wk->ev_seed_out, ss));
            HIPCHK(hipStreamWaitEvent(st, wk->ev_seed_out, 0));
        }
    }
    (void)hipEventRecord(wk->ev_probe[1], st);
    (void)hipEventRecord(wk->ev[2], st);
    {
        size_t tmp_bytes = 0;
        hipcub::DeviceScan::ExclusiveSum(nullptr, tmp_bytes, (unsigned long long *)wk->seed_cnt.p, (unsigned long long *)wk->seed_off.p, n + 1, st);
        ENS(scan_tmp, tmp_bytes + 256);
        HIPCHK(hipcub::DeviceScan::ExclusiveSum(wk->scan_tmp.p, tmp_bytes, (unsigned long long *)wk->seed_cnt.p, (unsigned long long *)wk->seed_off.p, n + 1, st));
    }
    {
        MailSpec ms{};
        ms.src[0] = (const unsigned int *)(wk->seed_off.as<uint64_t>() + n); ms.words[0] = 2;
        ms.src[1] = (const unsigned int *)ck.flags; ms.words[1] = 1;
        ms.src[2] = wk->queues.as<unsigned int>() + 31; ms.words[2] = 1;
        ms.src[3] = wk->queues.as<unsigned int>() + 34; ms.words[3] = 1;
        ms.src[4] = wk->queues.as<unsigned int>() + 35; ms.words[4] = 4;
        ms.n = 5;
        hipLaunchKernelGGL(k_mail, dim3(1), dim3(64), 0, st, ms, wk->h_mail);
    }
    HIPCHK(slx_wait_stream(st));
    unsigned long long S = 0;
    memcpy(&S, wk->h_mail, 8);
    const uint32_t fl0 = wk->h_mail[2];
    const unsigned int max_cnt = wk->h_mail[3], n_heavy_h = wk->h_mail[4];
    unsigned int n_p2_h = 0, n_long_h = 0, n_it_h = 0;
    unsigned int p2c[4] = {wk->h_mail[5], wk->h_mail[6], wk->h_mail[7], wk->h_mail[8]};
    n_p2_h = p2c[0]; n_it_h = p2c[2]; n_long_h = p2c[3];
    wk->cnt[0] += n_heavy_h; wk->cnt[1] += n_it_h; wk->cnt[2] += n_long_h; wk->cnt[3] += n_p2_h;
    if (getenv("SLX_DEBUG_SEED")) fprintf(stderr, "[seed] worker %d: %d reads, pass 2: %u single calls (%u of them one wave each) + %u whole reads (repeat filter k = %d), %u heavy\n", wk->id, n, n_it_h, n_long_h, n_p2_h, fm.rep ? fm.rep_k : 0, n_heavy_h);
    if (fl0) { *flags_out = fl0; return SLX_OK; }
    wk->max_seed_cnt = max_cnt;
    const size_t S1 = (size_t)S + 1;
    ENS(s_rbeg, S1 * 8); ENS(s_ql, S1 * sizeof(qp_t)); ENS(s_next, S1 * 4); ENS(c_pos, S1 * 8); ENS(c_head, S1 * 4); ENS(c_tail, S1 * 4);
    ENS(c_n, S1 * 4); ENS(c_rid, S1 * 4); ENS(c_w, S1 * 4); ENS(c_first, S1 * 4); ENS(c_kept, S1); ENS(ia, S1 * 4); ENS(ib, S1 * 4);
    ENS(ic, S1 * 4); ENS(srt, S1 * 8); ENS(regs, S1 * sizeof(DReg)); ENS(hits, S1 * sizeof(DHit));
    ENS(jobs, S1 * sizeof(DJob)); ENS(fast_list, S1 * 4); ENS(dp_list, S1 * 4); ENS(cig_lane_list, S1 * 4);
    ck.s_rbeg = wk->s_rbeg.as<int64_t>(); ck.s_ql = wk->s_ql.as<uint32_t>(); ck.s_next = wk->s_next.as<int32_t>();
    ck.c_pos = wk->c_pos.as<int64_t>(); ck.c_head = wk->c_head.as<int32_t>(); ck.c_tail = wk->c_tail.as<int32_t>();
    ck.c_n = wk->c_n.as<int32_t>(); ck.c_rid = wk->c_rid.as<int32_t>(); ck.c_w = wk->c_w.as<int32_t>();
    ck.c_first = wk->c_first.as<int32_t>(); ck.c_kept = wk->c_kept.as<int8_t>();
    ck.ia = wk->ia.as<int32_t>(); ck.ib = wk->ib.as<int32_t>(); ck.ic = wk->ic.as<int32_t>(); ck.srt = wk->srt.as<uint64_t>();
    ck.regs = wk->regs.as<DReg>(); ck.hits = wk->hits.as<DHit>();
    wk->last_S1 = S1;
    if (has_long) {
        ENS(s_score, S1 * 4); ENS(long_list, (size_t)n * 4);
        ck.s_score = wk->s_score.as<int32_t>();
        ck.long_stride = max_len + 8; ck.long_threads = n_threads;
        ENS(long_scratch, (size_t)n_threads * 2 * ck.long_stride * 4);
        ck.long_scratch = wk->long_scratch.as<int>();
        if (3 * (max_len + 8) * 4 > 64 * 1024) {
            ck.huge_stride = max_len + 8;
            ENS(huge_rows, (size_t)HUGE_BLOCKS * 3 * ck.huge_stride * 4);
            ck.huge_rows = wk->huge_rows.as<int>();
        }
    }
    (void)hipEventRecord(wk->ev[3], st);
    {
        unsigned int *q = wk->queues.as<unsigned int>();
        unsigned int *counts = q + 24;
        ENS(part_flag, (size_t)n * 4); ENS(part_pos, (size_t)n * 4); ENS(order_in, (size_t)n * 4); ENS(order_out, (size_t)n * 4);
        if (al->chain_lds) ENS(chain_left, (size_t)n * 4);
        {
            size_t tb = 0;
            HIPCHK(hipcub::DeviceScan::ExclusiveSum(nullptr, tb, wk->part_flag.as<unsigned int>(), wk->part_pos.as<unsigned int>(), n + 1, st));
            ENS(scan_tmp, tb + 256);
        }
        const bool dbg_on = getenv("SLX_DEBUG_SUB") != nullptr;
        if (dbg_on) (void)hipEventRecord(wk->dbg_ev[0], st);
        const bool hsort = al->heavy_sorted && al->heavy_seeds <= 0xfffff;
        if (!production) {
            if ((max_len > 704 && al->long_coop) || (max_len <= 704 && al->small_coop && n_heavy_h > 0)) {
                hipLaunchKernelGGL(k_part_flags, dim3((unsigned)((n + 255) / 256)), dim3(256), 0, st, wk->seed_cnt.as<unsigned long long>(), n,
                                   (unsigned int)al->heavy_seeds, wk->part_flag.as<unsigned int>());
                size_t tb = wk->scan_tmp.cap;
                HIPCHK(hipcub::DeviceScan::ExclusiveSum(wk->scan_tmp.p, tb, wk->part_flag.as<unsigned int>(), wk->part_pos.as<unsigned int>(), n, st));
                hipLaunchKernelGGL(k_part_scatter, dim3((unsigned)((n + 255) / 256)), dim3(256), 0, st, wk->part_flag.as<unsigned int>(),
                                   wk->part_pos.as<unsigned int>(), n, wk->order_in.as<int>(), wk->order_out.as<int>(), counts);
                launch_chain<I>(al, wk, ck, dopt, fm, st, wk->order_in.as<int>(), q, counts, n, spread > 1 ? seed_grid : grid, bs);
                launch_coop<I>(al, wk, ck, dopt, fm, st, q, counts, n, max_len > 704);
                hipLaunchKernelGGL(k_set_u32, dim3(1), dim3(1), 0, st, counts, (unsigned int)n);
            } else {
            hipLaunchKernelGGL(k_set_u32, dim3(1), dim3(1), 0, st, counts, (unsigned int)n);
            launch_chain<I>(al, wk, ck, dopt, fm, st, (const int *)nullptr, q, counts, n, spread > 1 ? seed_grid : grid, bs);
            }
            if (has_long) {
                hipLaunchKernelGGL(k_long_list, dim3((unsigned)((n + 255) / 256)), dim3(256), 0, st, ck, dopt, wk->long_list.as<int>(), q + 16);
                hipLaunchKernelGGL(k_flt_score, dim3((unsigned)std::min<int64_t>((int64_t)n * FLT_PARTS, 0x7fffffff)), dim3(64), 0, st, al->ref, ck, dopt, wk->long_list.as<int>(), q + 16);
                hipLaunchKernelGGL(k_flt_seeds, dim3(std::max(1, std::min(n, al->n_cu * 8))), dim3(64), 0, st, al->ref, ck, dopt, wk->long_list.as<int>(), q + 16, q + 17);
            }
            (void)hipEventRecord(wk->ev_probe[2], st);
            (void)hipEventRecord(wk->ev[4], st);
            if (max_len > 8192 && al->long_budget > 0 && al->long_predict) {
                ENS(first_off, ((size_t)n + 2) * 4);
                HIPCHK(hipMemsetAsync(wk->first_off.p, 0, ((size_t)n + 2) * 4, st));
                launch_tail<MAXQ_LONG>(al, wk, ck, dopt, q, counts, grid, bs, n, nullptr, nullptr, nullptr, nullptr, wk->first_off.as<unsigned int>(), 0u, (const DReg *)nullptr, true);
            }
            else if (max_len > 704) {
                const unsigned int top_cap = (unsigned int)std::min<uint64_t>((uint64_t)S1, 0x7fffffffu);
                ENS(first_tab, (size_t)top_cap * sizeof(DReg)); ENS(first_cnt, ((size_t)n + 2) * 4); ENS(first_off, ((size_t)n + 2) * 4);
                ENS(first_jobs, (size_t)top_cap * sizeof(FirstJob));
                HIPCHK(hipMemsetAsync(wk->first_cnt.p, 0, ((size_t)n + 2) * 4, st));
                hipLaunchKernelGGL(k_first_count, dim3((unsigned)((n + 255) / 256)), dim3(256), 0, st, ck, n, 0xffffffffu, wk->first_cnt.as<unsigned int>(), 0);
                size_t tb = wk->scan_tmp.cap;
                HIPCHK(hipcub::DeviceScan::ExclusiveSum(wk->scan_tmp.p, tb, wk->first_cnt.as<unsigned int>(), wk->first_off.as<unsigned int>(), n + 1, st));
                hipLaunchKernelGGL(k_first_prep, dim3(std::max(1, std::min(n / 128 + 1, al->n_cu * 12))), dim3(128), 0, st, al->ref, ck, dopt, n, wk->first_off.as<unsigned int>(),
                                   top_cap, wk->first_jobs.as<FirstJob>());
                const unsigned first_smem = ck.huge_rows ? 0u : (unsigned)(2 * ck.long_stride * 4);
                if (al->long_block && n <= al->long_block / 4 && max_len > 8192) {
                    unsigned int n_top_h = 0;
                    HIPCHK(hipMemcpyAsync(&n_top_h, wk->first_off.as<unsigned int>() + n, 4, hipMemcpyDeviceToHost, st));
                    HIPCHK(slx_wait_stream(st));
                    n_top_h = std::min(n_top_h, top_cap);
                    const bool sorted = n_top_h > 1 && sort_jobs_longest_first(wk, st, wk->first_jobs.as<FirstJob>(), nullptr, n_top_h);
                    if (n_top_h && launch_ext_jobs_seg(al, wk, ck, dopt, st, n_top_h, wk->first_jobs.as<FirstJob>(), wk->first_tab.as<DReg>(),
                                                       sorted ? (const unsigned int *)wk->job_val_out.as<unsigned int>() : (const unsigned int *)nullptr, first_smem)) {}
                    else
                    hipLaunchKernelGGL(k_ext_block, dim3(HUGE_BLOCKS), dim3(XB_THREADS), first_smem, st, al->ref, ck, dopt, wk->first_off.as<unsigned int>() + n, top_cap, q + 22,
                                       wk->first_jobs.as<FirstJob>(), wk->first_tab.as<DReg>(), sorted ? (const unsigned int *)wk->job_val_out.as<unsigned int>() : (const unsigned int *)nullptr,
                                       sorted ? (const unsigned int *)(wk->first_off.as<unsigned int>() + n) : (const unsigned int *)nullptr);
                }
                else
                hipLaunchKernelGGL(k_ext_first<MAXQ_LONG>, dim3(ck.huge_rows ? HUGE_BLOCKS : al->n_cu * 8), dim3(64), first_smem, st, al->ref, ck, dopt, n, wk->first_off.as<unsigned int>(),
                                   top_cap, q + 22, wk->first_jobs.as<FirstJob>(), wk->first_tab.as<DReg>(), (const unsigned int *)nullptr, (const unsigned int *)nullptr);
                launch_tail<MAXQ_LONG>(al, wk, ck, dopt, q, counts, grid, bs, n, nullptr, nullptr, nullptr, nullptr, wk->first_off.as<unsigned int>(), top_cap, wk->first_tab.as<DReg>());
            }
            else with_maxq(max_len, [&](auto mq) {
                launch_tail<decltype(mq)::value>(al, wk, ck, dopt, q, counts, grid, bs, n, nullptr, nullptr, nullptr, nullptr);
            });
        } else {
            hipLaunchKernelGGL(k_part_flags, dim3((unsigned)((n + 255) / 256)), dim3(256), 0, st, wk->seed_cnt.as<unsigned long long>(), n,
                               (unsigned int)al->heavy_seeds, wk->part_flag.as<unsigned int>());
            size_t tb = wk->scan_tmp.cap;
            HIPCHK(hipcub::DeviceScan::ExclusiveSum(wk->scan_tmp.p, tb, wk->part_flag.as<unsigned int>(), wk->part_pos.as<unsigned int>(), n, st));
            hipLaunchKernelGGL(k_part_scatter, dim3((unsigned)((n + 255) / 256)), dim3(256), 0, st, wk->part_flag.as<unsigned int>(),
                               wk->part_pos.as<unsigned int>(), n, wk->order_in.as<int>(), wk->order_out.as<int>(), counts);
            if (hsort && n_heavy_h > 1) {
                const unsigned int nh = n_heavy_h;
                ENS(order_key_in, (size_t)nh * 4); ENS(order_key_out, (size_t)nh * 4); ENS(order_tmp, (size_t)nh * 4);
                hipLaunchKernelGGL(k_heavy_keys, dim3((nh + 255) / 256), dim3(256), 0, st, wk->seed_cnt.as<unsigned long long>(), wk->order_out.as<int>(), nh,
                                   wk->order_key_in.as<unsigned int>());
                size_t tb2 = 0;
                HIPCHK(hipcub::DeviceRadixSort::SortPairsDescending(nullptr, tb2, wk->order_key_in.as<unsigned int>(), wk->order_key_out.as<unsigned int>(),
                                                                    wk->order_out.as<int>(), wk->order_tmp.as<int>(), (int)nh, 0, 20, st));
                ENS(sort_tmp, tb2 + 256);
                HIPCHK(hipcub::DeviceRadixSort::SortPairsDescending(wk->sort_tmp.p, tb2, wk->order_key_in.as<unsigned int>(), wk->order_key_out.as<unsigned int>(),
                                                                    wk->order_out.as<int>(), wk->order_tmp.as<int>(), (int)nh, 0, 20, st));
                HIPCHK(hipMemcpyAsync(wk->order_out.p, wk->order_tmp.p, (size_t)nh * 4, hipMemcpyDeviceToDevice, st));
            }
            hipLaunchKernelGGL(k_set_u32, dim3(1), dim3(1), 0, st, counts + 2, (unsigned int)n);
            const int *light = wk->order_in.as<int>();
            if (al->chain_sorted && wk->order_bin.ensure((size_t)n * 4) == SLX_OK && wk->bin_cnt.ensure(512) == SLX_OK && hipMemsetAsync(wk->bin_cnt.p, 0, 512, st) == hipSuccess) {
                const dim3 gbn((unsigned)((n + 255) / 256));
                unsigned int *bins = wk->bin_cnt.as<unsigned int>();
                hipLaunchKernelGGL(k_nreg_bin_count<unsigned long long>, gbn, dim3(256), 0, st, light, (const unsigned int *)counts, (const unsigned long long *)wk->seed_cnt.as<unsigned long long>(), bins);
                hipLaunchKernelGGL(k_nreg_bin_scan, dim3(1), dim3(64), 0, st, bins);
                hipLaunchKernelGGL(k_nreg_bin_scatter<unsigned long long>, gbn, dim3(256), 0, st, light, (const unsigned int *)counts, (const unsigned long long *)wk->seed_cnt.as<unsigned long long>(), bins,
                                   wk->order_bin.as<int>());
                light = wk->order_bin.as<int>();
            } else (void)hipGetLastError();
            launch_chain<I>(al, wk, ck, dopt, fm, st, light, q, counts, n, grid, bs);
            launch_coop<I>(al, wk, ck, dopt, fm, st, q, counts, n);
            (void)hipEventRecord(wk->ev_probe[2], st);
            if (use_cand) {
                const int nh = (int)n_heavy_h;
                const unsigned gb = (unsigned)((nh + 255) / 256) + 1;
                HIPCHK(hipMemsetAsync(wk->cand_cnt.p, 0, ((size_t)nh + 2) * 8, st));
                unsigned int *slot_cnt = wk->cand_cnt.as<unsigned int>(), *job_cnt = slot_cnt + (nh + 2);
                unsigned int *slot_off = wk->cand_off.as<unsigned int>(), *job_off = slot_off + (nh + 2);
                int amax = 0;
                for (int i = 0; i < 25; ++i) amax = std::max(amax, (int)opt->mat[i]);
                amax = std::max(amax, opt->a);
                const int lane_cols = max_len - std::min(opt->min_seed_len, max_len) + 2 + al->lane_pad;
                const bool lane_narrow = al->lane_narrow && amax * max_len < 256;
                const bool lanes = (al->cand_lanes > 0 || (al->cand_lanes < 0 && n <= CAND_REP_AUTO_READS)) && max_len <= 704 && (lane_narrow ? LaneNarrow::bytes(lane_cols) : LaneWide::bytes(lane_cols)) <= 64 * 1024 &&
                                   (int64_t)amax * max_len < LANE_SCORE_LIMIT;
                const int cand_rep = lanes ? 0 : (al->cand_rep >= 0 ? al->cand_rep : (n <= CAND_REP_AUTO_READS ? 75 : 0));
                for (int pass = cand_rep > 0 ? 1 : 0; pass >= 0; --pass)
                    hipLaunchKernelGGL(k_cand_count, dim3(gb), dim3(256), 0, st, ck, wk->order_out.as<int>(), counts + 1, slot_cnt, job_cnt,
                                       (unsigned int)(lanes ? al->cand_lane_seeds : al->cand_seeds), (hsort && !lanes) ? (unsigned int)al->cand_top : 0xffffffffu,
                                       (unsigned int)cand_rep, q + 30, (unsigned int)al->cand_rep_max, pass, lanes ? 1 : CAND_PART);
                tb = wk->scan_tmp.cap;
                HIPCHK(hipcub::DeviceScan::ExclusiveSum(wk->scan_tmp.p, tb, slot_cnt, slot_off, nh + 1, st));
                hipLaunchKernelGGL(k_cand_base, dim3(gb), dim3(256), 0, st, wk->order_out.as<int>(), counts + 1, slot_off, (unsigned int)al->cand_cap,
                                   wk->cand_base.as<int32_t>(), job_cnt);
                tb = wk->scan_tmp.cap;
                HIPCHK(hipcub::DeviceScan::ExclusiveSum(wk->scan_tmp.p, tb, job_cnt, job_off, nh + 1, st));
                const int gc = al->n_cu * 32;
                if (lanes) {
                    const size_t max_jobs = std::min<size_t>((size_t)al->cand_cap, S1);
                    ENS(lane_jobs, max_jobs * sizeof(LaneJob));
                    auto go = [&](auto mq) {
                        constexpr int MAXQ = decltype(mq)::value;
                        hipLaunchKernelGGL(k_cand_lane_prep<MAXQ>, dim3(std::max(1, std::min(nh, al->n_cu * 16))), dim3(64), 0, st, al->ref, ck, dopt, wk->order_out.as<int>(), counts + 1,
                                           job_off, wk->lane_jobs.as<LaneJob>());
                        if (lane_narrow) hipLaunchKernelGGL(k_ext_lanes<LaneNarrow>, dim3(al->n_cu * 8), dim3(64), LaneNarrow::bytes(lane_cols), st, al->ref, ck, dopt, counts + 1, job_off,
                                                            q + 14, wk->lane_jobs.as<LaneJob>(), wk->cand.as<DReg>(), lane_cols);
                        else hipLaunchKernelGGL(k_ext_lanes<LaneWide>, dim3(al->n_cu * 4), dim3(64), LaneWide::bytes(lane_cols), st, al->ref, ck, dopt, counts + 1, job_off, q + 14,
                                                wk->lane_jobs.as<LaneJob>(), wk->cand.as<DReg>(), lane_cols);
                    };
                    with_maxq(max_len, go);
                } else
                with_maxq(max_len, [&](auto mq) {
                    hipLaunchKernelGGL(k_extend_cand<decltype(mq)::value>, dim3(gc), dim3(64), 0, st, al->ref, ck, dopt, wk->order_out.as<int>(), counts + 1,
                                       job_off, q + 14, wk->cand.as<DReg>());
                });
            }
            if (hsort && al->ext_split) {
                const unsigned int top_cap = (unsigned int)std::min<uint64_t>((uint64_t)n + std::min<uint64_t>((uint64_t)S1, (uint64_t)n), 0x7fffffffu);
                ENS(first_tab, (size_t)top_cap * sizeof(DReg)); ENS(first_cnt, ((size_t)n + 2) * 4); ENS(first_off, ((size_t)n + 2) * 4); ENS(fb_list, (size_t)n * 4);
                unsigned int *n_fb = q + 20, *ext_tot = q + 21;
                HIPCHK(hipMemsetAsync(wk->first_cnt.p, 0, ((size_t)n + 2) * 4, st));
                hipLaunchKernelGGL(k_first_count, dim3((unsigned)((n + 255) / 256)), dim3(256), 0, st, ck, n, (unsigned int)al->heavy_seeds, wk->first_cnt.as<unsigned int>(),
                                   al->top_heavy);
                tb = wk->scan_tmp.cap;
                HIPCHK(hipcub::DeviceScan::ExclusiveSum(wk->scan_tmp.p, tb, wk->first_cnt.as<unsigned int>(), wk->first_off.as<unsigned int>(), n + 1, st));
                const int gf = al->n_cu * 32;
                ENS(first_jobs, (size_t)top_cap * sizeof(FirstJob));
                if (al->first_diag) ENS(first_dp, (size_t)top_cap * 4);
                int fl_amax = 0;
                for (int i = 0; i < 25; ++i) fl_amax = std::max(fl_amax, (int)opt->mat[i]);
                fl_amax = std::max(fl_amax, opt->a);
                const int fl_cols = max_len - std::min(opt->min_seed_len, max_len) + 2 + al->lane_pad;
                const bool fl_narrow = al->lane_narrow && fl_amax * max_len < 256;
                const bool first_lanes = al->first_lanes && al->first_diag && max_len <= 704 && (fl_narrow ? LaneNarrow::bytes(fl_cols) : LaneWide::bytes(fl_cols)) <= 64 * 1024 &&
                                         (int64_t)fl_amax * max_len < LANE_SCORE_LIMIT;
                if (first_lanes) {
                    ENS(first_sorted, (size_t)top_cap * 4); ENS(first_bins, 1024);
                    HIPCHK(hipMemsetAsync(wk->first_bins.p, 0, 512, st));
                    wk->first_lanes_ran = true;
                }
                hipLaunchKernelGGL(k_first_prep, dim3(std::max(1, std::min(n / 128 + 1, al->n_cu * 12))), dim3(128), 0, st, al->ref, ck, dopt, n, wk->first_off.as<unsigned int>(),
                                   top_cap, wk->first_jobs.as<FirstJob>());
                with_maxq(max_len, [&](auto mq) {
                    constexpr int MAXQ = decltype(mq)::value;
                    if (al->first_diag) {
                        hipLaunchKernelGGL(k_first_diag, dim3((top_cap + 255) / 256), dim3(256), 0, st, al->ref, ck, dopt, n, wk->first_off.as<unsigned int>(), top_cap,
                                           wk->first_jobs.as<FirstJob>(), wk->first_tab.as<DReg>(), wk->first_dp.as<unsigned int>(), q + 40);
                    }
                    if (first_lanes) {
                        unsigned int *bins = wk->first_bins.as<unsigned int>(), *sorted = wk->first_sorted.as<unsigned int>();
                        const FirstJob *fj = wk->first_jobs.as<FirstJob>();
                        hipLaunchKernelGGL(k_first_bin_count, dim3(al->n_cu * 4), dim3(256), 0, st, fj, (const unsigned int *)wk->first_dp.as<unsigned int>(), (const unsigned int *)(q + 40), max_len, bins);
                        hipLaunchKernelGGL(k_first_bin_scan, dim3(1), dim3(1), 0, st, bins);
                        hipLaunchKernelGGL(k_first_bin_scatter, dim3(al->n_cu * 4), dim3(256), 0, st, fj, (const unsigned int *)wk->first_dp.as<unsigned int>(), (const unsigned int *)(q + 40), max_len, bins, sorted);
                        if (fl_narrow) hipLaunchKernelGGL(k_first_lanes<LaneNarrow>, dim3(al->n_cu * 8), dim3(64), LaneNarrow::bytes(fl_cols), st, al->ref, ck, dopt, q + 22, fj, wk->first_tab.as<DReg>(),
                                                          (const unsigned int *)sorted, (const unsigned int *)(q + 40), fl_cols, q + 54);
                        else hipLaunchKernelGGL(k_first_lanes<LaneWide>, dim3(al->n_cu * 4), dim3(64), LaneWide::bytes(fl_cols), st, al->ref, ck, dopt, q + 22, fj, wk->first_tab.as<DReg>(),
                                                (const unsigned int *)sorted, (const unsigned int *)(q + 40), fl_cols, q + 54);
                    } else
                    hipLaunchKernelGGL(k_ext_first<MAXQ>, dim3(gf), dim3(64), 0, st, al->ref, ck, dopt, n, wk->first_off.as<unsigned int>(), top_cap, q + 22,
                                       wk->first_jobs.as<FirstJob>(), wk->first_tab.as<DReg>(), al->first_diag ? wk->first_dp.as<unsigned int>() : (const unsigned int *)nullptr, q + 40);
#ifdef EXT_STATS
                    ext_stats_print(st, "cand + ext_first", n, wk->first_off.as<unsigned int>() + n);
#endif
                    hipLaunchKernelGGL(k_ext_replay<MAXQ>, dim3(grid), dim3(bs), 0, st, al->ref, ck, dopt, n, (unsigned int)al->heavy_seeds, wk->first_off.as<unsigned int>(),
                                       top_cap, wk->first_tab.as<DReg>(), q + 23, wk->fb_list.as<int>(), n_fb);
                });
                hipLaunchKernelGGL(k_add_u32, dim3(1), dim3(1), 0, st, counts + 1, n_fb, ext_tot);
                (void)hipEventRecord(wk->ev[4], st);
                with_maxq(max_len, [&](auto mq) {
                    launch_tail<decltype(mq)::value>(al, wk, ck, dopt, q, counts + 2, grid, bs, n, wk->fb_list.as<int>(), wk->order_out.as<int>(), counts + 1, ext_tot,
                                                     al->top_reuse ? wk->first_off.as<unsigned int>() : nullptr, top_cap, wk->first_tab.as<DReg>());
                });
            } else {
                (void)hipEventRecord(wk->ev[4], st);
                with_maxq(max_len, [&](auto mq) {
                    if (hsort) launch_tail<decltype(mq)::value>(al, wk, ck, dopt, q, counts + 2, grid, bs, n, wk->order_in.as<int>(), wk->order_out.as<int>(), counts + 1, nullptr);
                    else launch_tail<decltype(mq)::value>(al, wk, ck, dopt, q, counts + 2, grid, bs, n, nullptr, nullptr, nullptr, nullptr);
                });
            }
        }
    }
    (void)hipEventRecord(wk->ev[6], st);
    hipLaunchKernelGGL(k_hit_counts, dim3((unsigned)((n + 255) / 256)), dim3(256), 0, st, ck, wk->cig_cnt.as<unsigned long long>());
    {
        hipcub::TransformInputIterator<unsigned long long, CvtI32U64, const int *> it(wk->n_hit.as<int>(), CvtI32U64());
        size_t tb = 0;
        hipcub::DeviceScan::ExclusiveSum(nullptr, tb, it, wk->hit_off_c.as<unsigned long long>(), n + 1, st);
        ENS(scan_tmp, tb + 256);
        HIPCHK(hipcub::DeviceScan::ExclusiveSum(wk->scan_tmp.p, tb, it, wk->hit_off_c.as<unsigned long long>(), n + 1, st));
        size_t tb2 = 0;
        hipcub::DeviceScan::ExclusiveSum(nullptr, tb2, wk->cig_cnt.as<unsigned long long>(), wk->cig_off_c.as<unsigned long long>(), n + 1, st);
        ENS(scan_tmp, tb2 + 256);
        HIPCHK(hipcub::DeviceScan::ExclusiveSum(wk->scan_tmp.p, tb2, wk->cig_cnt.as<unsigned long long>(), wk->cig_off_c.as<unsigned long long>(), n + 1, st));
    }
    unsigned long long Hc = 0, Cc = 0;
    int m_hits, m_cig, m_flags, m_defer, m_big, m_chain, m_walk, m_first = -1;
    {
        MailSpec ms{};
        int at = 0;
        auto part = [&](const unsigned int *src, int words) {
            if (ms.n >= SLX_MAIL_PARTS || at + words > 64) return -1;
            ms.src[ms.n] = src; ms.words[ms.n] = words; ++ms.n;
            at += words;
            return at - words;
        };
        m_hits = part((const unsigned int *)(wk->hit_off_c.as<unsigned long long>() + n), 2);
        m_cig = part((const unsigned int *)(wk->cig_off_c.as<unsigned long long>() + n), 2);
        m_flags = part((const unsigned int *)ck.flags, 1);
        m_defer = part(wk->queues.as<unsigned int>() + 46, 1);
        m_big = part(wk->queues.as<unsigned int>() + 48, 1);
        m_chain = part(wk->queues.as<unsigned int>() + 50, 2);
        m_walk = part(wk->queues.as<unsigned int>() + 55, 2);
        if (wk->first_lanes_ran) m_first = part(wk->queues.as<unsigned int>() + 54, 1);
        if (m_hits < 0 || m_cig < 0 || m_flags < 0 || m_defer < 0 || m_big < 0 || m_chain < 0 || m_walk < 0 || (wk->first_lanes_ran && m_first < 0)) {
            slx_set_error("run_chunk: more counters than k_mail has parts (SLX_MAIL_PARTS)");
            return SLX_EINTERNAL;
        }
        hipLaunchKernelGGL(k_mail, dim3(1), dim3(64), 0, st, ms, wk->h_mail);
    }
    HIPCHK(slx_wait_stream(st));
    memcpy(&Hc, wk->h_mail + m_hits, 8); memcpy(&Cc, wk->h_mail + m_cig, 8);
    const uint32_t fl = wk->h_mail[m_flags];
    wk->fin_stat[0] += wk->h_mail[m_defer]; wk->fin_stat[1] += wk->h_mail[m_big];
    if (fl) { *flags_out = fl; return SLX_OK; }
    wk->chain_stat[0] += wk->h_mail[m_chain]; wk->chain_stat[1] += wk->h_mail[m_chain + 1];
    wk->walk_stat += wk->h_mail[m_walk];
    wk->exit_stat += wk->h_mail[m_walk + 1];
    if (m_first >= 0) wk->first_stat += wk->h_mail[m_first];
    const size_t H = (size_t)*hit_base + Hc, C = (size_t)*cig_base + Cc;
#define GROW(buf, bytes, keep) if ((rc = wk->buf.grow((size_t)(bytes), (size_t)(keep), st)) != SLX_OK) return rc
    GROW(o_rid, (H + 1) * 4, *hit_base * 4); GROW(o_pos, (H + 1) * 8, *hit_base * 8); GROW(o_flag, (H + 1) * 2, *hit_base * 2);
    GROW(o_mapq, (H + 1), *hit_base); GROW(o_score, (H + 1) * 4, *hit_base * 4); GROW(o_nm, (H + 1) * 4, *hit_base * 4);
    GROW(o_na, (H + 1) * 4, *hit_base * 4); GROW(o_ncig, (H + 1) * 4, *hit_base * 4); GROW(o_cig_off, (H + 2) * 8, *hit_base * 8);
    GROW(o_cigar, (C + 1) * 4, *cig_base * 4);
    if (ck.sam_mode) { GROW(o_xa, (H + 1) * 4, *hit_base * 4); GROW(o_sub, (H + 1) * 4, *hit_base * 4); }
    HitsSoA so;
    so.hit_off = wk->o_hit_off.as<int64_t>(); so.rid = wk->o_rid.as<int32_t>(); so.pos = wk->o_pos.as<int64_t>();
    so.flag = wk->o_flag.as<uint16_t>(); so.mapq = wk->o_mapq.as<uint8_t>(); so.score = wk->o_score.as<int32_t>();
    so.nm = wk->o_nm.as<int32_t>(); so.na = wk->o_na.as<int32_t>(); so.n_cigar_ops = wk->o_ncig.as<int32_t>();
    so.cig_off = wk->o_cig_off.as<int64_t>(); so.cigar = wk->o_cigar.as<uint32_t>();
    so.xa_parent = ck.sam_mode ? wk->o_xa.as<int32_t>() : nullptr; so.sub = ck.sam_mode ? wk->o_sub.as<int32_t>() : nullptr;
    hipLaunchKernelGGL(k_compact, dim3((unsigned)((n + 255) / 256)), dim3(256), 0, st, ck, wk->hit_off_c.as<unsigned long long>(),
                       wk->cig_off_c.as<unsigned long long>(), so, r0 - part_lo, *hit_base, *cig_base);
    (void)hipEventRecord(wk->ev[7], st);
    HIPCHK(hipGetLastError());
    HIPCHK(slx_wait_stream(st));
    for (int i = 0; i < 7; ++i) {
        float ms = 0;
        if (hipEventElapsedTime(&ms, wk->ev[i], wk->ev[i + 1]) == hipSuccess) wk->stage_ms[i] += ms;
    }
    for (int i = 0; i < 3; ++i) {
        float ms = 0;
        if (hipEventElapsedTime(&ms, wk->ev_probe[2 * i], wk->ev_probe[2 * i + 1]) == hipSuccess) wk->probe_ms[i] += ms;
    }
    {
        hipEvent_t a[3] = {wk->ev[3], wk->ev_probe[3], wk->ev_probe[5]}, b[3] = {wk->ev_probe[2], wk->ev_probe[4], wk->ev[6]};
        for (int i = 0; i < 3; ++i) {
            float ms = 0;
            if (hipEventElapsedTime(&ms, a[i], b[i]) == hipSuccess) wk->probe_ms[3 + i] += ms;
        }
    }
    if (ck.dbg_cyc && ck.dbg_stage == 3) {
        unsigned long long c6[32];
        HIPCHK(hipMemcpy(c6, wk->dbg_cyc.p, 256, hipMemcpyDeviceToHost));
        fprintf(stderr, "[seed12m] calls with min_intv <= 2: %llu, %.1f backward steps each; others: %llu, %.1f each; by length < 64 / < 256 / < 1024 / more: %llu (%.3g steps), %llu (%.3g), %llu (%.3g), %llu (%.3g); longest %llu\n",
                c6[16], c6[16] ? (double)c6[17] / (double)c6[16] : 0., c6[18], c6[18] ? (double)c6[19] / (double)c6[18] : 0., c6[20], (double)c6[21], c6[22], (double)c6[23], c6[24], (double)c6[25],
                c6[26], (double)c6[27], c6[30]);
        {
            std::vector<unsigned long long> life((size_t)grid * 2);
            HIPCHK(hipMemcpy(life.data(), wk->dbg_cyc.as<unsigned long long>() + 64, life.size() * 8, hipMemcpyDeviceToHost));
            std::vector<unsigned long long> lv;
            for (unsigned long long v : life) if (v) lv.push_back(v);
            std::sort(lv.begin(), lv.end());
            if (!lv.empty()) {
                fprintf(stderr, "[seed12m] wave lifetimes (cycle-counter ticks), %zu waves: min %.3g  p10 %.3g  p50 %.3g  p90 %.3g  p99 %.3g  max %.3g\n", lv.size(), (double)lv[0],
                        (double)lv[lv.size() / 10], (double)lv[lv.size() / 2], (double)lv[lv.size() * 9 / 10], (double)lv[lv.size() * 99 / 100], (double)lv.back());
            }
        }
        fprintf(stderr, "[seed12m] lanes per round by phase: fetch %.1f init %.1f start %.1f fwd %.1f dir %.1f row %.1f bwd %.1f done %.1f\n", (double)c6[8] / (double)c6[4],
                (double)c6[9] / (double)c6[4], (double)c6[10] / (double)c6[4], (double)c6[11] / (double)c6[4], (double)c6[12] / (double)c6[4], (double)c6[13] / (double)c6[4],
                (double)c6[14] / (double)c6[4], (double)c6[15] / (double)c6[4]);
        fprintf(stderr, "[seed12m] forward loop: %.4g wave-steps, %.1f lanes active; backward loop: %.4g wave-steps, %.1f lanes active; %.4g rounds, %.4g with events; direct loop: %.4g wave-steps (32 bases each), %.1f lanes active; %d reads\n",
                (double)c6[0], (double)c6[1] / (double)(c6[0] ? c6[0] : 1), (double)c6[2], (double)c6[3] / (double)(c6[2] ? c6[2] : 1), (double)c6[4], (double)c6[5], (double)c6[6], (double)c6[7] / (double)(c6[6] ? c6[6] : 1), n);
    } else if (ck.dbg_cyc) {
        std::vector<unsigned long long> cyc((size_t)n * 4), sc((size_t)n);
        std::vector<int> nch((size_t)n), nrg((size_t)n), lrep((size_t)n);
        HIPCHK(hipMemcpy(lrep.data(), wk->l_rep.p, (size_t)n * 4, hipMemcpyDeviceToHost));
        HIPCHK(hipMemcpy(cyc.data(), wk->dbg_cyc.p, (size_t)n * 32, hipMemcpyDeviceToHost));
        HIPCHK(hipMemcpy(sc.data(), wk->seed_cnt.p, (size_t)n * 8, hipMemcpyDeviceToHost));
        HIPCHK(hipMemcpy(nch.data(), wk->n_chain.p, (size_t)n * 4, hipMemcpyDeviceToHost));
        HIPCHK(hipMemcpy(nrg.data(), wk->n_reg.p, (size_t)n * 4, hipMemcpyDeviceToHost));
        std::vector<int> ord((size_t)n);
        for (int i = 0; i < n; ++i) ord[(size_t)i] = i;
        const int top = std::min(n, 12);
        std::partial_sort(ord.begin(), ord.begin() + top, ord.end(), [&](int a, int b) { return cyc[(size_t)a] > cyc[(size_t)b]; });
        unsigned long long tot = 0, tot_heavy = 0;
        unsigned long long ph[3] = {0, 0, 0};
        for (int i = 0; i < n; ++i) {
            tot += cyc[(size_t)i];
            if (sc[(size_t)i] >= (unsigned long long)al->heavy_seeds) tot_heavy += cyc[(size_t)i];
            for (int k = 0; k < 3; ++k) ph[k] += cyc[(size_t)(k + 1) * (size_t)n + (size_t)i];
        }
        float ext_ms = 0;
        (void)hipEventElapsedTime(&ext_ms, wk->ev[4], wk->ev[5]);
        fprintf(stderr, "[ext phases] sort %.3g  covered tests %.3g  extend+store %.3g ticks; extension stage %.1f ms\n", (double)ph[0], (double)ph[1], (double)ph[2], ext_ms);
        {
            const int lim[6] = {2, 8, 48, 128, 256, 640};
            for (int b = 0; b < 6; ++b) {
                long cnt = 0; unsigned long long cy = 0, a = 0, bb = 0, c = 0;
                for (int i = 0; i < n; ++i)
                    if (nrg[(size_t)i] >= lim[b] && (b == 5 || nrg[(size_t)i] < lim[b + 1])) {
                        ++cnt; cy += cyc[(size_t)i]; a += cyc[(size_t)n + i]; bb += cyc[2 * (size_t)n + i]; c += cyc[3 * (size_t)n + i];
                    }
                fprintf(stderr, "[regions >= %d] reads %ld  ticks %.3g (A %.3g B %.3g C %.3g)\n", lim[b], cnt, (double)cy, (double)a, (double)bb, (double)c);
            }
        }
        {
            const int lb[5] = {0, 1, 50, 100, 140};
            for (int b = 0; b < 5; ++b) {
                long cnt = 0; unsigned long long cy = 0;
                for (int i = 0; i < n; ++i)
                    if (nrg[(size_t)i] >= 256 && lrep[(size_t)i] >= lb[b] && (b == 4 || lrep[(size_t)i] < lb[b + 1])) { ++cnt; cy += cyc[(size_t)i]; }
                fprintf(stderr, "[>= 256 regions, l_rep >= %d] reads %ld  mean ticks %.3g\n", lb[b], cnt, cnt ? (double)cy / (double)cnt : 0.0);
            }
        }
        fprintf(stderr, "[ext cycles] n=%d total=%.3g (100 MHz ticks) heavy share=%.3f\n", n, (double)tot, tot ? (double)tot_heavy / (double)tot : 0.0);
        for (int i = 0; i < top; ++i) {
            const size_t r = (size_t)ord[(size_t)i];
            fprintf(stderr, "  read %zu: %.3g ticks (A %.3g, B %.3g, C %.3g; stage 1: sort, covered tests, extend+store; stage 2: sort by end, dedup/patch, second sort)  seeds=%llu chains=%d regions=%d l_rep=%d\n", r, (double)cyc[r],
                    (double)cyc[(size_t)n + r], (double)cyc[2 * (size_t)n + r], (double)cyc[3 * (size_t)n + r], sc[r], nch[r], nrg[r], lrep[r]);
        }
    }
    if (getenv("SLX_DEBUG_SUB")) {
        const char *nm[5] = {"chain", "extend", "regs", "cig", "hits"};
        fprintf(stderr, "[worker %d n=%d]", wk->id, n);
        for (int i = 0; i < 5; ++i) { float ms = -1; (void)hipEventElapsedTime(&ms, wk->dbg_ev[i], wk->dbg_ev[i + 1]); fprintf(stderr, " %s=%.1f", nm[i], ms); }
        float tot = -1; (void)hipEventElapsedTime(&tot, wk->dbg_ev[0], wk->dbg_ev[5]);
        fprintf(stderr, " total=%.1f\n", tot);
    }
    wk->last_ck = ck; wk->last_valid = true; wk->last_wide = sizeof(I) == 8;
    *hit_base += (int64_t)Hc;
    *cig_base += (int64_t)Cc;
    *flags_out = 0;
    return SLX_OK;
#undef ENS
#undef GROW
}
```

Measured before the change: 78.02 million.

## Route near-diagonal first extensions to a narrow-band ring lane kernel

New measurement: 80.19 million (median of 6 runs). 2.8% higher.

```diff
diff --git a/seqlib_amd/csrc/dev_ext_lane.h b/seqlib_amd/csrc/dev_ext_lane.h
--- a/seqlib_amd/csrc/dev_ext_lane.h
+++ b/seqlib_amd/csrc/dev_ext_lane.h
@@ -31,7 +31,7 @@
 
 template <typename L>
 __device__ DReg lane_extend_core(const DevRef &R, const slx_opt &opt, const MatRows &mr, const uint8_t *query, int l_query, int s_qbeg, int s_len,
-                                 int64_t s_rbeg, int64_t rmax0, int64_t rmax1, int rid, float frac_rep, L &eh, int row_exit, unsigned int &n_exit)
+                                 int64_t s_rbeg, int64_t rmax0, int64_t rmax1, int rid, float frac_rep, L &eh, int row_exit, unsigned int &n_exit, int wband0 = -1, int wband1 = -1)
 {
     DReg a;
     a.rb = a.re = 0; a.qb = a.qe = 0; a.sub = a.csub = a.sub_n = 0; a.seedcov = 0; a.secondary = 0;
@@ -43,8 +43,8 @@
     const int64_t re0 = s_rbeg + s_len;
     a.qe = l_query; a.re = re0;
     LaneSide sd[2];
-    sd[0].qlen = s_qbeg; sd[0].tlen = (int)(s_rbeg - rmax0); sd[0].q0 = s_qbeg - 1; sd[0].t0 = s_rbeg - 1; sd[0].end_bonus = opt.pen_clip5;
-    sd[1].qlen = l_query - qe; sd[1].tlen = (int)(rmax1 - re0); sd[1].q0 = qe; sd[1].t0 = re0; sd[1].end_bonus = opt.pen_clip3;
+    sd[0].qlen = s_qbeg; sd[0].tlen = (int)(s_rbeg - rmax0); sd[0].q0 = s_qbeg - 1; sd[0].t0 = s_rbeg - 1; sd[0].end_bonus = opt.pen_clip5; sd[0].wband = wband0;
+    sd[1].qlen = l_query - qe; sd[1].tlen = (int)(rmax1 - re0); sd[1].q0 = qe; sd[1].t0 = re0; sd[1].end_bonus = opt.pen_clip3; sd[1].wband = wband1;
     LaneBases bases{R, query, {0, -1}};
     lane_rows_extend(sd, s_len * opt.a, opt, mr, eh, bases, [&](int side, const LaneRes &er) {
         if (side == 0) {
@@ -171,21 +171,26 @@
     lane_exits_add(ck.ext_exits, exit_cnt, lane);
 }
 
-__device__ __forceinline__ int first_job_bin(const FirstJob &j, int max_len)
+__device__ __forceinline__ int first_job_band(const FirstJob &j, int side) { return (int)((side ? (unsigned int)j.pad >> 16 : (unsigned int)j.pad) & 0xffffu) - 1; }
+__device__ __forceinline__ int first_job_bin(const FirstJob &j, int max_len, int by_band)
 {
     const int left = j.s_qbeg, right = j.l_query - j.s_qbeg - j.s_len;
-    const float w = sqrtf((float)(left * left + right * right));
+    float w;
+    if (by_band) {
+        const int b0 = first_job_band(j, 0), b1 = first_job_band(j, 1);
+        w = (float)(left * (2 * (b0 > 0 ? b0 : 0) + 1) + right * (2 * (b1 > 0 ? b1 : 0) + 1)) / (float)(2 * EXT_NARROW_CAP + 1);
+    } else w = sqrtf((float)(left * left + right * right));
     int b = (int)(w * 64.f / (float)(max_len > 0 ? max_len : 1));
     b = b > 63 ? 63 : (b < 0 ? 0 : b);
     return 63 - b;
 }
-__global__ void __launch_bounds__(256) k_first_bin_count(const FirstJob *jobs, const unsigned int *dp_list, const unsigned int *n_dp, int max_len, unsigned int *bins)
+__global__ void __launch_bounds__(256) k_first_bin_count(const FirstJob *jobs, const unsigned int *dp_list, const unsigned int *n_dp, int max_len, unsigned int *bins, int by_band)
 {
     __shared__ unsigned int s[64];
     if (threadIdx.x < 64) s[threadIdx.x] = 0;
     __syncthreads();
     const unsigned int n = *n_dp;
-    for (unsigned int t = blockIdx.x * blockDim.x + threadIdx.x; t < n; t += gridDim.x * blockDim.x) atomicAdd(&s[first_job_bin(jobs[dp_list[t]], max_len)], 1u);
+    for (unsigned int t = blockIdx.x * blockDim.x + threadIdx.x; t < n; t += gridDim.x * blockDim.x) atomicAdd(&s[first_job_bin(jobs[dp_list[t]], max_len, by_band)], 1u);
     __syncthreads();
     if (threadIdx.x < 64 && s[threadIdx.x]) atomicAdd(&bins[threadIdx.x], s[threadIdx.x]);
 }
@@ -193,7 +198,7 @@
 {
     if (blockIdx.x == 0 && threadIdx.x == 0) { unsigned int acc = 0; for (int b = 0; b < 64; ++b) { bins[64 + b] = acc; acc += bins[b]; } }
 }
-__global__ void __launch_bounds__(256) k_first_bin_scatter(const FirstJob *jobs, const unsigned int *dp_list, const unsigned int *n_dp, int max_len, unsigned int *bins, unsigned int *out)
+__global__ void __launch_bounds__(256) k_first_bin_scatter(const FirstJob *jobs, const unsigned int *dp_list, const unsigned int *n_dp, int max_len, unsigned int *bins, unsigned int *out, int by_band)
 {
     __shared__ unsigned int s_cnt[64], s_base[64];
     const unsigned int n = *n_dp;
@@ -203,7 +208,7 @@
         const unsigned int t = t0 + threadIdx.x;
         int b = -1;
         unsigned int job = 0, my = 0;
-        if (t < n) { job = dp_list[t]; b = first_job_bin(jobs[job], max_len); my = atomicAdd(&s_cnt[b], 1u); }
+        if (t < n) { job = dp_list[t]; b = first_job_bin(jobs[job], max_len, by_band); my = atomicAdd(&s_cnt[b], 1u); }
         __syncthreads();
         if (threadIdx.x < 64 && s_cnt[threadIdx.x]) s_base[threadIdx.x] = atomicAdd(&bins[64 + threadIdx.x], s_cnt[threadIdx.x]);
         __syncthreads();
@@ -231,7 +236,8 @@
         if (t < n_jobs) {
             const unsigned int job = list[t];
             const FirstJob j = jobs[job];
-            const DReg a = lane_extend_core<L>(R, opt, mr, ck.codes + j.q_off, j.l_query, j.s_qbeg, j.s_len, j.s_rbeg, j.rmax0, j.rmax1, j.rid, j.frac_rep, row, ck.ext_row_exit, exit_cnt);
+            const DReg a = lane_extend_core<L>(R, opt, mr, ck.codes + j.q_off, j.l_query, j.s_qbeg, j.s_len, j.s_rbeg, j.rmax0, j.rmax1, j.rid, j.frac_rep, row, ck.ext_row_exit, exit_cnt,
+                                                 first_job_band(j, 0), first_job_band(j, 1));
             first[job] = a;
         }
         if (lane == 0) atomicAdd(n_ran, n_jobs - base < (unsigned int)WAVE ? n_jobs - base : (unsigned int)WAVE);
@@ -240,8 +246,9 @@
 }
 
 template <typename QF, typename TF>
-__device__ __forceinline__ bool lane_diag_extend(int qlen, QF qf, int tlen, TF tf, const slx_opt &o, const MatRows &mr, int amax, int h0, ExtResult &out)
-{
+__device__ __forceinline__ bool lane_diag_extend(int qlen, QF qf, int tlen, TF tf, const slx_opt &o, const MatRows &mr, int amax, int h0, int loss_stop, ExtResult &out, int &loss_out)
+{
+    loss_out = -1;
     if (tlen < qlen || qlen > 3 * WAVE || qlen < 1) return false;
     if ((long long)h0 + (long long)qlen * amax >= (1 << 22)) return false;
     const int oe_del = o.o_del + o.e_del, oe_ins = o.o_ins + o.e_ins;
@@ -253,28 +260,37 @@
         const int row4 = t == 0 ? mr.q4[0] : t == 1 ? mr.q4[1] : t == 2 ? mr.q4[2] : mr.q4[3];
         const int sc = q < 4 ? __builtin_amdgcn_sbfe((int)rowp, (uint32_t)q << 3, 8u) : row4;
         loss += amax - sc;
-        if (loss > oe - 1) return false;
+        if (loss > loss_stop) return false;
         run += sc;
         if (run > best) { best = run; best_p = p; }
     }
-    if (h0 <= loss) return false;
+    loss_out = loss;
+    if (loss > oe - 1 || h0 <= loss) return false;
     out.score = best; out.qle = best_p + 1; out.tle = best_p + 1; out.gtle = qlen; out.gscore = run; out.max_off = 0;
     return true;
 }
 
-__global__ void __launch_bounds__(256) k_first_diag(DevRef R, Chunk ck, DevOpt dopt, int n, const unsigned int *first_off, unsigned int cap, const FirstJob *jobs, DReg *first,
-                                                    unsigned int *dp_list, unsigned int *n_dp)
-{
-    const slx_opt &opt = dopt.o;
-    const MatRows mr = make_matrows(opt.mat);
-    int amax = 0;
-    for (int i = 0; i < 25; ++i) amax = amax > opt.mat[i] ? amax : opt.mat[i];
-    unsigned int n_jobs = first_off[n];
-    if (n_jobs > cap) n_jobs = cap;
-    const unsigned int job = blockIdx.x * blockDim.x + threadIdx.x;
-    if (job >= n_jobs) return;
+__device__ __forceinline__ int first_side_band(const slx_opt &o, int amax, int loss, int h0_lower, int qlen, int tlen, int end_bonus, bool &dp_side)
+{
+    dp_side = false;
+    const int oe_del = o.o_del + o.e_del, oe_ins = o.o_ins + o.e_ins;
+    const int oe = oe_del < oe_ins ? oe_del : oe_ins;
+    if (o.e_ins <= 0 || o.e_del <= 0) return -1;
+    const int lim = ext_eff_band(o, qlen, amax, end_bonus, 0x3fffffff);
+    int band = -1;
+    if (loss >= 0) {
+        band = ext_narrow_band(o, amax, loss > oe ? loss : oe, h0_lower, qlen, tlen, o.w < lim ? o.w : lim);
+        dp_side = band >= 0 && loss > oe - 1;
+    }
+    if (band < 0 && lim <= EXT_NARROW_CAP) band = EXT_NARROW_CAP;
+    return band;
+}
+
+__device__ __forceinline__ bool first_diag_job(const DevRef &R, const Chunk &ck, const slx_opt &opt, const MatRows &mr, int amax, FirstJob *jobs, unsigned int job, DReg *first, int narrow,
+                                               bool &all, unsigned int &n_dp_sides)
+{
     const FirstJob j = jobs[job];
-    if (j.l_query <= 0) return;
+    if (j.l_query <= 0) return false;
     const uint8_t *codes = ck.codes;
     QWin qw; qw.bits = 0; qw.chunk = 0xffffffffu;
     RWin rw; rw.bits = 0; rw.chunk = -1;
@@ -284,39 +300,96 @@
     a.score = a.truesc = -1; a.rid = j.rid;
     const int aw_ext = ((opt.w >> 1) + (opt.w >> 2)) > 0 ? opt.w : opt.w << 1;
     int aw0 = opt.w, aw1 = opt.w;
-    bool ok = true;
+    const int oe_del = opt.o_del + opt.e_del, oe_ins = opt.o_ins + opt.e_ins;
+    const int oe = oe_del < oe_ins ? oe_del : oe_ins;
+    int loss_stop = oe - 1;
+    if (narrow && opt.o_del >= 0 && opt.o_ins >= 0 && opt.e_del > 0 && opt.e_ins > 0) {
+        const long long sd = (long long)opt.o_del + (long long)(EXT_NARROW_CAP + 1) * opt.e_del, si = (long long)opt.o_ins + (long long)(EXT_NARROW_CAP + 1) * opt.e_ins;
+        const long long st = (sd < si ? sd : si) - 1;
+        loss_stop = st > loss_stop ? (st < (1 << 20) ? (int)st : (1 << 20)) : loss_stop;
+    }
+    bool ok0 = true, ok1 = true;
+    int loss0 = -1, loss1 = -1;
     const int s_qbeg = j.s_qbeg, s_len = j.s_len, l_query = j.l_query;
     const int64_t s_rbeg = j.s_rbeg;
+    const int qe = s_qbeg + s_len;
+    const int64_t re0 = s_rbeg + s_len;
     if (s_qbeg) {
         aw0 = aw_ext;
         ExtResult er;
-        ok = lane_diag_extend(s_qbeg, [&](int p) { return q_at(codes, j.q_off + (uint64_t)(s_qbeg - 1 - p), qw); }, (int)(s_rbeg - j.rmax0),
-                              [&](int t) { return text_at(R, s_rbeg - 1 - t, rw); }, opt, mr, amax, s_len * opt.a, er);
-        if (ok) {
+        ok0 = lane_diag_extend(s_qbeg, [&](int p) { return q_at(codes, j.q_off + (uint64_t)(s_qbeg - 1 - p), qw); }, (int)(s_rbeg - j.rmax0),
+                               [&](int t) { return text_at(R, s_rbeg - 1 - t, rw); }, opt, mr, amax, s_len * opt.a, loss_stop, er, loss0);
+        if (ok0) {
             a.score = er.score;
             if (er.gscore <= 0 || er.gscore <= a.score - opt.pen_clip5) { a.qb = s_qbeg - er.qle; a.rb = s_rbeg - er.tle; a.truesc = a.score; }
             else { a.qb = 0; a.rb = s_rbeg - er.gtle; a.truesc = er.gscore; }
         }
     } else { a.score = a.truesc = s_len * opt.a; a.qb = 0; a.rb = s_rbeg; }
-    if (ok) {
-        if (s_qbeg + s_len != l_query) {
+    const int h0_right = ok0 ? a.score : s_len * opt.a;
+    if (ok0 || narrow) {
+        if (qe != l_query) {
             aw1 = aw_ext;
-            const int sc0 = a.score, qe = s_qbeg + s_len;
-            const int64_t re0 = s_rbeg + s_len;
+            const int sc0 = a.score;
             ExtResult er;
-            ok = lane_diag_extend(l_query - qe, [&](int p) { return q_at(codes, j.q_off + (uint64_t)(qe + p), qw); }, (int)(j.rmax1 - re0),
-                                  [&](int t) { return text_at(R, re0 + t, rw); }, opt, mr, amax, sc0, er);
-            if (ok) {
+            ok1 = lane_diag_extend(l_query - qe, [&](int p) { return q_at(codes, j.q_off + (uint64_t)(qe + p), qw); }, (int)(j.rmax1 - re0),
+                                   [&](int t) { return text_at(R, re0 + t, rw); }, opt, mr, amax, h0_right, loss_stop, er, loss1);
+            if (ok0 && ok1) {
                 a.score = er.score;
                 if (er.gscore <= 0 || er.gscore <= a.score - opt.pen_clip3) { a.qe = qe + er.qle; a.re = re0 + er.tle; a.truesc += a.score - sc0; }
                 else { a.qe = l_query; a.re = re0 + er.gtle; a.truesc += er.gscore - sc0; }
             }
         } else { a.qe = l_query; a.re = s_rbeg + s_len; }
     }
-    if (ok) {
+    if (ok0 && ok1) {
         a.w = aw0 > aw1 ? aw0 : aw1;
         a.seedlen0 = s_len;
         a.frac_rep = j.frac_rep;
         first[job] = a;
-    } else dp_list[wave_fetch_inc(n_dp)] = job;
-}
+        return false;
+    }
+    if (narrow) {
+        bool dp0 = false, dp1 = false;
+        const int b0 = s_qbeg ? first_side_band(opt, amax, loss0, s_len * opt.a, s_qbeg, (int)(s_rbeg - j.rmax0), opt.pen_clip5, dp0) : -1;
+        const int b1 = qe != l_query ? first_side_band(opt, amax, loss1, h0_right, l_query - qe, (int)(j.rmax1 - re0), opt.pen_clip3, dp1) : -1;
+        jobs[job].pad = (int)((unsigned int)(b0 + 1) | (unsigned int)(b1 + 1) << 16);
+        all = (!s_qbeg || b0 >= 0) && (qe == l_query || b1 >= 0);
+        n_dp_sides = (unsigned int)dp0 + (unsigned int)dp1;
+    }
+    return true;
+}
+
+__global__ void __launch_bounds__(256) k_first_diag(DevRef R, Chunk ck, DevOpt dopt, int n, const unsigned int *first_off, unsigned int cap, FirstJob *jobs, DReg *first,
+                                                    unsigned int *dp_list, unsigned int *n_dp, int narrow, unsigned int *nar_list, unsigned int *nar_stat)
+{
+    const slx_opt &opt = dopt.o;
+    const MatRows mr = make_matrows(opt.mat);
+    int amax = 0;
+    for (int i = 0; i < 25; ++i) amax = amax > opt.mat[i] ? amax : opt.mat[i];
+    unsigned int n_jobs = first_off[n];
+    if (n_jobs > cap) n_jobs = cap;
+    const unsigned int job = blockIdx.x * blockDim.x + threadIdx.x;
+    bool all = false;
+    unsigned int sides = 0;
+    const bool dp = job < n_jobs && first_diag_job(R, ck, opt, mr, amax, jobs, job, first, narrow, all, sides);
+    __shared__ unsigned int s_cnt[4][3], s_base[2];
+    const int wv = threadIdx.x >> 6, ln = threadIdx.x & (WAVE - 1);
+    const bool to_nar = dp && all && nar_list != nullptr, to_dp = dp && !to_nar;
+    const unsigned long long m_dp = __ballot(to_dp), m_nar = __ballot(to_nar);
+    const unsigned int w_all = (unsigned int)__popcll(__ballot(dp && all));
+    const unsigned int w_sides = (unsigned int)__builtin_amdgcn_readlane(dpp_incl_add_scan((int)sides), WAVE - 1);
+    if (ln == 0) { s_cnt[wv][0] = (unsigned int)__popcll(m_dp); s_cnt[wv][1] = (unsigned int)__popcll(m_nar); s_cnt[wv][2] = w_all | w_sides << 16; }
+    __syncthreads();
+    if (threadIdx.x == 0) {
+        unsigned int d = 0, a = 0, n_all = 0, n_sides = 0;
+        for (int w = 0; w < 4; ++w) {
+            unsigned int t = s_cnt[w][0]; s_cnt[w][0] = d; d += t;
+            t = s_cnt[w][1]; s_cnt[w][1] = a; a += t;
+            n_all += s_cnt[w][2] & 0xffffu; n_sides += s_cnt[w][2] >> 16;
+        }
+        s_base[0] = d ? atomicAdd(n_dp, d) : 0u;
+        s_base[1] = (n_all | n_sides) ? (unsigned int)atomicAdd((unsigned long long *)nar_stat, (unsigned long long)n_all | (unsigned long long)n_sides << 32) : 0u;
+    }
+    __syncthreads();
+    if (to_dp) dp_list[s_base[0] + s_cnt[wv][0] + __builtin_amdgcn_mbcnt_hi((uint32_t)(m_dp >> 32), __builtin_amdgcn_mbcnt_lo((uint32_t)m_dp, 0u))] = job;
+    if (to_nar) nar_list[s_base[1] + s_cnt[wv][1] + __builtin_amdgcn_mbcnt_hi((uint32_t)(m_nar >> 32), __builtin_amdgcn_mbcnt_lo((uint32_t)m_nar, 0u))] = job;
+}
diff --git a/seqlib_amd/csrc/dev_lane_rows.h b/seqlib_amd/csrc/dev_lane_rows.h
--- a/seqlib_amd/csrc/dev_lane_rows.h
+++ b/seqlib_amd/csrc/dev_lane_rows.h
@@ -38,7 +38,34 @@
 }
 LROW_FN bool ext_row_done(int U, int max, int gscore, int end_bonus) { return (end_bonus >= 0 && U <= max - end_bonus) || ext_tail_done(U, max, gscore); }
 
+#define EXT_NARROW_CAP 14
+template <typename O>
+LROW_FN int ext_narrow_band(const O &o, int amax, int L, int h0_lower, int qlen, int tlen, int w_eff)
+{
+    if (o.o_del < 0 || o.o_ins < 0 || o.e_del <= 0 || o.e_ins <= 0 || amax <= 0) return -1;
+    if (qlen < 1 || qlen > tlen) return -1;
+    const int oe_del = o.o_del + o.e_del, oe_ins = o.o_ins + o.e_ins;
+    if (L <= (oe_del < oe_ins ? oe_del : oe_ins) - 1) return -1;
+    if (h0_lower <= L) return -1;
+    if (o.zdrop > 0 && 2ll * L > o.zdrop) return -1;
+    const int wd = L >= o.o_del ? (L - o.o_del) / o.e_del : -1, wi = L >= o.o_ins ? (L - o.o_ins) / o.e_ins : -1;
+    const int w = wd > wi ? wd : wi;
+    return w >= 0 && w < w_eff && w <= EXT_NARROW_CAP ? w : -1;
+}
+template <typename O>
+LROW_FN int ext_eff_band(const O &o, int qlen, int amax, int end_bonus, int w)
+{
+    const int xi = qlen * amax + end_bonus - o.o_ins, xd = qlen * amax + end_bonus - o.o_del;
+    int max_ins = o.e_ins ? xi / o.e_ins + 1 : (xi > 0 ? 0x7fffffff : 1);
+    max_ins = max_ins > 1 ? max_ins : 1;
+    w = w < max_ins ? w : max_ins;
+    int max_del = o.e_del ? xd / o.e_del + 1 : (xd > 0 ? 0x7fffffff : 1);
+    max_del = max_del > 1 ? max_del : 1;
+    return w < max_del ? w : max_del;
+}
+
 struct LaneWide {
+    static constexpr bool ring = false;
     uint32_t *eh;
     static LROW_M size_t bytes(int cols) { return (size_t)cols * WAVE * 4; }
     LROW_M void init(uint32_t *base, int, int lane) { eh = base + lane; }
@@ -51,6 +78,7 @@
     static LROW_M bool zero(uint32_t v) { return (v & 0x0fffffffu) == 0; }
 };
 struct LaneNarrow {
+    static constexpr bool ring = false;
     uint16_t *eh;
     uint32_t *qa;
     static LROW_M size_t bytes(int cols) { return (size_t)cols * WAVE * 2 + (size_t)((cols + 7) / 8) * WAVE * 4; }
@@ -70,7 +98,29 @@
     static LROW_M bool zero(uint32_t v) { return v == 0; }
 };
 
-struct LaneSide { int qlen, tlen, q0, end_bonus; int64_t t0; };
+#define LANE_RING_COLS 32
+struct LaneRing {
+    static constexpr bool ring = true;
+    uint16_t *eh;
+    uint32_t *qa;
+    static LROW_M size_t bytes(int cols) { return (size_t)LANE_RING_COLS * WAVE * 2 + (size_t)((cols + 7) / 8) * WAVE * 4; }
+    LROW_M void init(uint32_t *base, int, int lane) { eh = (uint16_t *)base + lane; qa = base + (size_t)LANE_RING_COLS * WAVE / 2 + lane; }
+    LROW_M void put_all(int j, int h, int e, int q)
+    {
+        if (j < LANE_RING_COLS) eh[j * WAVE] = (uint16_t)(h | e << 8);
+        uint32_t w = (j & 7) ? qa[(j >> 3) * WAVE] : 0u;
+        w |= (uint32_t)q << ((j & 7) * 4);
+        qa[(j >> 3) * WAVE] = w;
+    }
+    LROW_M uint32_t get(int j) const { return eh[(j & (LANE_RING_COLS - 1)) * WAVE]; }
+    LROW_M int q_of(uint32_t, int j) const { return (int)((qa[(j >> 3) * WAVE] >> ((j & 7) * 4)) & 7u); }
+    static LROW_M int h_of(uint32_t v) { return (int)(v & 0xffu); }
+    static LROW_M int e_of(uint32_t v) { return (int)(v >> 8); }
+    LROW_M void put(int j, int h, int e, uint32_t) { eh[(j & (LANE_RING_COLS - 1)) * WAVE] = (uint16_t)(h | e << 8); }
+    static LROW_M bool zero(uint32_t v) { return v == 0; }
+};
+
+struct LaneSide { int qlen, tlen, q0, end_bonus; int64_t t0; int wband = -1; };
 struct LaneRes { int score, qle, tle, gtle, gscore, max_off, aw; };
 
 template <typename L, typename F, typename O, typename MR, typename D>
@@ -88,6 +138,7 @@
     const int apos = amax > 0 ? amax : 0;
     int64_t t0 = 0;
     int max = 0, max_i = -1, max_j = -1, max_ie = -1, gscore = -1, max_off = 0, beg = 0, end = 0, i = 0;
+    int top = 0;
     while (side < 2) {
         if (fresh) {
             fresh = false;
@@ -100,18 +151,15 @@
                 const int h = j == 0 ? h0 : (v > 0 ? v : 0);
                 row.put_all(j, h, 0, j < qlen ? fetch.q(q0 + dir * j) : 0);
             }
-            w = aw;
-            int max_ins = (int)((double)(qlen * amax + end_bonus - o_ins) / e_ins + 1.);
-            max_ins = max_ins > 1 ? max_ins : 1;
-            w = w < max_ins ? w : max_ins;
-            int max_del = (int)((double)(qlen * amax + end_bonus - o_del) / e_del + 1.);
-            max_del = max_del > 1 ? max_del : 1;
-            w = w < max_del ? w : max_del;
+            w = ext_eff_band(o, qlen, amax, end_bonus, aw);
+            const int wband = side ? s[1].wband : s[0].wband;
+            if (wband >= 0) w = w < wband ? w : wband;
             tail_top = ext_tail_bound0(o, qlen, h0, amax);
             exit_ok = row_exit != EXT_ROW_EXIT_OFF && ext_row_exit_ok(o, qlen, w, h0);
             exit_bonus = row_exit == EXT_ROW_EXIT_RELAXED ? end_bonus : -1;
             max = h0;
             max_i = -1; max_j = -1; max_ie = -1; gscore = -1; max_off = 0; beg = 0; end = qlen; i = 0;
+            top = qlen < LANE_RING_COLS - 1 ? qlen : LANE_RING_COLS - 1;
         }
         bool stop = i >= tlen || (i >= qlen && ext_tail_done(tail_top - (i - qlen) * e_del, max, gscore));
         if (!stop) {
@@ -122,6 +170,9 @@
             if (beg < i - w) beg = i - w;
             if (end > i + w + 1) end = i + w + 1;
             if (end > qlen) end = qlen;
+            if (L::ring) {
+                for (; top < end; ++top) { const int v = h0 - oe_ins - top * e_ins; row.put(top + 1, v > 0 ? v : 0, 0, 0u); }
+            }
             int h1 = 0;
             if (beg == 0) { h1 = h0 - (o_del + e_del * (i + 1)); if (h1 < 0) h1 = 0; }
             const int hb = h1;
diff --git a/seqlib_amd/csrc/slx_align.hip b/seqlib_amd/csrc/slx_align.hip
--- a/seqlib_amd/csrc/slx_align.hip
+++ b/seqlib_amd/csrc/slx_align.hip
@@ -513,6 +513,7 @@
     else if (!strcmp(key, "top_reuse")) al->top_reuse = value != 0;
     else if (!strcmp(key, "walk_stage")) al->walk_stage = value != 0;
     else if (!strcmp(key, "ext_row_exit")) al->ext_row_exit = value != 0;
+    else if (!strcmp(key, "ext_narrow")) { if (value < 0 || value > 3) return SLX_EINVAL; al->ext_narrow = (int)value; }
     else if (!strcmp(key, "p2_items")) al->p2_items = value != 0;
     else if (!strcmp(key, "p2_coop")) al->p2_coop = value != 0;
     else if (!strcmp(key, "p2_items_cap")) al->p2_items_cap = (int)value;
@@ -601,6 +602,13 @@
         if (!strcmp(key, "first_lane_jobs")) {
             long long v = 0;
             auto take = [&](const slx_aligner *a) { for (const Worker *wk : a->workers) v += (long long)wk->first_stat; };
+            if (al->is_group) for (const slx_aligner *sub : al->subs) take(sub); else take(al);
+            return v;
+        }
+        if (!strcmp(key, "ext_narrow_sides") || !strcmp(key, "ext_narrow_jobs")) {
+            long long v = 0;
+            const int which = key[11] == 'j';
+            auto take = [&](const slx_aligner *a) { for (const Worker *wk : a->workers) v += (long long)wk->narrow_stat[which]; };
             if (al->is_group) for (const slx_aligner *sub : al->subs) take(sub); else take(al);
             return v;
         }
@@ -739,6 +747,7 @@
     wk->first_stat = 0;
     wk->walk_stat = 0;
     wk->exit_stat = 0;
+    wk->narrow_stat[0] = wk->narrow_stat[1] = 0;
     int rc;
     const int64_t n_part = r_hi - r_lo;
     if ((rc = wk->o_hit_off.ensure(((size_t)n_part + 1) * 8)) != SLX_OK) return rc;
diff --git a/seqlib_amd/csrc/slx_align_types.h b/seqlib_amd/csrc/slx_align_types.h
--- a/seqlib_amd/csrc/slx_align_types.h
+++ b/seqlib_amd/csrc/slx_align_types.h
@@ -75,6 +75,7 @@
     DevBuf chain_left;
     DevBuf order_bin, bin_cnt;
     DevBuf defer_list, hits_big;
+    DevBuf first_nar, first_nar_sorted;
     DevBuf first_sorted, first_bins;
     DevBuf p2mask, p2list, p2items, p2long, lane_jobs, first_dp, cig_lane_list;
     DevBuf job_key_in, job_key_out, job_val_in, job_val_out, job_sort_tmp;
@@ -89,6 +90,7 @@
     unsigned long long first_stat = 0;
     bool first_lanes_ran = false;
     unsigned long long walk_stat = 0;
+    unsigned long long narrow_stat[2] = {0, 0};
     unsigned long long exit_stat = 0;
     unsigned int pseg_stat = 0;
     unsigned int gseg_stat[3] = {0, 0, 0};
@@ -117,7 +119,7 @@
                &c_pos, &c_head, &c_tail, &c_n, &c_rid, &c_w, &c_first, &c_kept, &ia, &ib, &ic, &srt, &regs, &hits, &n_chain, &n_reg, &n_hit,
                &na, &frac_rep, &zarena, &cigpool, &counters, &lists, &hit_cnt, &cig_cnt, &hit_off_c, &cig_off_c, &order_key_in,
                &order_key_out, &order_in, &order_out, &queues, &sort_tmp, &jobs, &fast_list, &dp_list, &part_flag, &part_pos, &cand, &cand_base,
-               &cand_cnt, &cand_off, &dbg_cyc, &order_tmp, &first_tab, &first_cnt, &first_off, &fb_list, &first_jobs, &len_stat, &s_score, &long_list, &long_scratch, &huge_rows, &p2mask, &p2list, &p2items, &p2long, &lane_jobs, &first_dp, &first_sorted, &first_bins, &cig_lane_list, &defer_list, &hits_big, &order_bin, &bin_cnt, &chain_left, &guard_cnt, &snap_ia, &snap_regs, &snap_nreg,
+               &cand_cnt, &cand_off, &dbg_cyc, &order_tmp, &first_tab, &first_cnt, &first_off, &fb_list, &first_jobs, &len_stat, &s_score, &long_list, &long_scratch, &huge_rows, &p2mask, &p2list, &p2items, &p2long, &lane_jobs, &first_dp, &first_sorted, &first_bins, &first_nar, &first_nar_sorted, &cig_lane_list, &defer_list, &hits_big, &order_bin, &bin_cnt, &chain_left, &guard_cnt, &snap_ia, &snap_regs, &snap_nreg,
                &memo_idx, &memo_jobs, &memo_tab, &round_list, &todo_a, &todo_b, &spec_cnt, &seed3_buf, &job_key_in, &job_key_out, &job_val_in, &job_val_out, &job_sort_tmp, &pseg_jobs, &pseg_idx, &pseg_cnt, &gseg_jobs, &gseg_units, &gseg_wrec, &gseg_wout, &gseg_scratch, &gseg_cnt, &xseg_jobs, &xseg_state, &xseg_units, &xseg_out, &xseg_wrec, &xseg_wout, &xseg_scratch, &xseg_cnt,
                &o_hit_off, &o_rid, &o_pos, &o_flag, &o_mapq, &o_score, &o_nm, &o_na, &o_ncig, &o_cig_off, &o_cigar, &o_xa, &o_sub};
         for (auto &e : ev) e = nullptr;
@@ -193,6 +195,7 @@
     int top_reuse = 1;
     int walk_stage = 1;
     int ext_row_exit = 1;
+    int ext_narrow = 1;
     int seed_free_cus = 0;
     int stream_prio = 0;
     int n_workers = 3;
diff --git a/seqlib_amd/csrc/slx_chunk.inc b/seqlib_amd/csrc/slx_chunk.inc
--- a/seqlib_amd/csrc/slx_chunk.inc
+++ b/seqlib_amd/csrc/slx_chunk.inc
@@ -885,9 +885,14 @@
                 const bool fl_narrow = al->lane_narrow && fl_amax * max_len < 256;
                 const bool first_lanes = al->first_lanes && al->first_diag && max_len <= 704 && (fl_narrow ? LaneNarrow::bytes(fl_cols) : LaneWide::bytes(fl_cols)) <= 64 * 1024 &&
                                          (int64_t)fl_amax * max_len < LANE_SCORE_LIMIT;
+                const int narrow = first_lanes ? al->ext_narrow : 0;
+                const bool ring = (narrow == 1 || narrow == 3) && fl_narrow;
+                const int by_band = narrow == 1;
+                const int ring_cu = 16;
                 if (first_lanes) {
                     ENS(first_sorted, (size_t)top_cap * 4); ENS(first_bins, 1024);
-                    HIPCHK(hipMemsetAsync(wk->first_bins.p, 0, 512, st));
+                    HIPCHK(hipMemsetAsync(wk->first_bins.p, 0, 1024, st));
+                    if (ring) { ENS(first_nar, (size_t)top_cap * 4); ENS(first_nar_sorted, (size_t)top_cap * 4); }
                     wk->first_lanes_ran = true;
                 }
                 hipLaunchKernelGGL(k_first_prep, dim3(std::max(1, std::min(n / 128 + 1, al->n_cu * 12))), dim3(128), 0, st, al->ref, ck, dopt, n, wk->first_off.as<unsigned int>(),
@@ -896,18 +901,28 @@
                     constexpr int MAXQ = decltype(mq)::value;
                     if (al->first_diag) {
                         hipLaunchKernelGGL(k_first_diag, dim3((top_cap + 255) / 256), dim3(256), 0, st, al->ref, ck, dopt, n, wk->first_off.as<unsigned int>(), top_cap,
-                                           wk->first_jobs.as<FirstJob>(), wk->first_tab.as<DReg>(), wk->first_dp.as<unsigned int>(), q + 40);
+                                           wk->first_jobs.as<FirstJob>(), wk->first_tab.as<DReg>(), wk->first_dp.as<unsigned int>(), q + 40, narrow,
+                                           ring ? wk->first_nar.as<unsigned int>() : (unsigned int *)nullptr, q + 58);
                     }
                     if (first_lanes) {
                         unsigned int *bins = wk->first_bins.as<unsigned int>(), *sorted = wk->first_sorted.as<unsigned int>();
                         const FirstJob *fj = wk->first_jobs.as<FirstJob>();
-                        hipLaunchKernelGGL(k_first_bin_count, dim3(al->n_cu * 4), dim3(256), 0, st, fj, (const unsigned int *)wk->first_dp.as<unsigned int>(), (const unsigned int *)(q + 40), max_len, bins);
+                        hipLaunchKernelGGL(k_first_bin_count, dim3(al->n_cu * 4), dim3(256), 0, st, fj, (const unsigned int *)wk->first_dp.as<unsigned int>(), (const unsigned int *)(q + 40), max_len, bins, 0);
                         hipLaunchKernelGGL(k_first_bin_scan, dim3(1), dim3(1), 0, st, bins);
-                        hipLaunchKernelGGL(k_first_bin_scatter, dim3(al->n_cu * 4), dim3(256), 0, st, fj, (const unsigned int *)wk->first_dp.as<unsigned int>(), (const unsigned int *)(q + 40), max_len, bins, sorted);
+                        hipLaunchKernelGGL(k_first_bin_scatter, dim3(al->n_cu * 4), dim3(256), 0, st, fj, (const unsigned int *)wk->first_dp.as<unsigned int>(), (const unsigned int *)(q + 40), max_len, bins, sorted, 0);
                         if (fl_narrow) hipLaunchKernelGGL(k_first_lanes<LaneNarrow>, dim3(al->n_cu * 8), dim3(64), LaneNarrow::bytes(fl_cols), st, al->ref, ck, dopt, q + 22, fj, wk->first_tab.as<DReg>(),
                                                           (const unsigned int *)sorted, (const unsigned int *)(q + 40), fl_cols, q + 54);
                         else hipLaunchKernelGGL(k_first_lanes<LaneWide>, dim3(al->n_cu * 4), dim3(64), LaneWide::bytes(fl_cols), st, al->ref, ck, dopt, q + 22, fj, wk->first_tab.as<DReg>(),
                                                 (const unsigned int *)sorted, (const unsigned int *)(q + 40), fl_cols, q + 54);
+                        if (ring) {
+                            const unsigned int *nar = wk->first_nar.as<unsigned int>();
+                            unsigned int *nbins = bins + 128, *nsorted = wk->first_nar_sorted.as<unsigned int>();
+                            hipLaunchKernelGGL(k_first_bin_count, dim3(al->n_cu * 4), dim3(256), 0, st, fj, nar, (const unsigned int *)(q + 58), max_len, nbins, by_band);
+                            hipLaunchKernelGGL(k_first_bin_scan, dim3(1), dim3(1), 0, st, nbins);
+                            hipLaunchKernelGGL(k_first_bin_scatter, dim3(al->n_cu * 4), dim3(256), 0, st, fj, nar, (const unsigned int *)(q + 58), max_len, nbins, nsorted, by_band);
+                            hipLaunchKernelGGL(k_first_lanes<LaneRing>, dim3(al->n_cu * ring_cu), dim3(64), LaneRing::bytes(fl_cols), st, al->ref, ck, dopt, q + 60, fj, wk->first_tab.as<DReg>(),
+                                               (const unsigned int *)nsorted, (const unsigned int *)(q + 58), fl_cols, q + 54);
+                        }
                     } else
                     hipLaunchKernelGGL(k_ext_first<MAXQ>, dim3(gf), dim3(64), 0, st, al->ref, ck, dopt, n, wk->first_off.as<unsigned int>(), top_cap, q + 22,
                                        wk->first_jobs.as<FirstJob>(), wk->first_tab.as<DReg>(), al->first_diag ? wk->first_dp.as<unsigned int>() : (const unsigned int *)nullptr, q + 40);
@@ -962,7 +977,7 @@
         m_defer = part(wk->queues.as<unsigned int>() + 46, 1);
         m_big = part(wk->queues.as<unsigned int>() + 48, 1);
         m_chain = part(wk->queues.as<unsigned int>() + 50, 2);
-        m_walk = part(wk->queues.as<unsigned int>() + 55, 2);
+        m_walk = part(wk->queues.as<unsigned int>() + 55, 5);
         if (wk->first_lanes_ran) m_first = part(wk->queues.as<unsigned int>() + 54, 1);
         if (m_hits < 0 || m_cig < 0 || m_flags < 0 || m_defer < 0 || m_big < 0 || m_chain < 0 || m_walk < 0 || (wk->first_lanes_ran && m_first < 0)) {
             slx_set_error("run_chunk: more counters than k_mail has parts (SLX_MAIL_PARTS)");
@@ -978,6 +993,7 @@
     wk->chain_stat[0] += wk->h_mail[m_chain]; wk->chain_stat[1] += wk->h_mail[m_chain + 1];
     wk->walk_stat += wk->h_mail[m_walk];
     wk->exit_stat += wk->h_mail[m_walk + 1];
+    wk->narrow_stat[0] += wk->h_mail[m_walk + 4]; wk->narrow_stat[1] += wk->h_mail[m_walk + 3];
     if (m_first >= 0) wk->first_stat += wk->h_mail[m_first];
     const size_t H = (size_t)*hit_base + Hc, C = (size_t)*cig_base + Cc;
 #define GROW(buf, bytes, keep) if ((rc = wk->buf.grow((size_t)(bytes), (size_t)(keep), st)) != SLX_OK) return rc
```
